# wangxuanx/Face-Diffusion-Model

Measured on AMD Instinct MI355X. Metric: animated frames/sec (1000-step DDPM, VOCASET FDM) at 1/2/4/8 MI355X, higher is better.
Workload: dtype bf16; 1 GPU; cfg2: vocaset FDM, 4 clips/GPU x 200 latent frames, 1000-step DDPM, random-init weights, synthetic audio-encoder features, Philox noise; global_batch=4, latent_frames=200, diffusion_steps=1000, parallelism=clip-shard x1

## Files before the change

### face-diffusion-model_amd/csrc/attention.hpp

```cpp
#pragma once
#include "common.hpp"
#include "../../include/fdm_hip.h"

namespace fdm {

template <typename T> __device__ __forceinline__ float fexp(float x) {
  if constexpr (is_fast16<T>::value) return __builtin_amdgcn_exp2f(x);
  else return expf(x);
}

template <typename T, int HD> constexpr bool attn_streamed() { return Opnd<T>::NP == 2 && HD == 256; }

template <typename T, int HD, int QS, bool RAG = false>
__global__ __launch_bounds__(256, (attn_streamed<T, HD>() ? 1 : 2)) void attn_kernel(const void* pQ, const void* pKp, const void* pVp, int p_q_lo_off, int p_kv_lo_off, int pL, int pB, int pH, int p_ldq,
                                                                                     int pLpad, const fdm_attn_args p) {
  using E = typename Opnd<T>::E;
  constexpr int NP = Opnd<T>::NP;
  constexpr float SCL = Opnd<T>::SCALE;
  constexpr int EPC = 16 / (int)sizeof(E);
  constexpr int NKS = HD / (4 * EPC);
  constexpr int KT = 4 * EPC;
  constexpr int NSUB = KT / 16;
  constexpr int NC = HD / 16;
  constexpr int BQ = 16 * QS;
// ... 162 lines not shown
          pf = __builtin_bit_cast(u32x4, pb);
        } else {
          pf = __builtin_bit_cast(u32x4, sc[0]);
        }
#pragma unroll
        for (int c = 0; c < NC; ++c) Mma<T>::run(o[u][c], vf[c][0], pf);
      } else {
        typedef __attribute__((ext_vector_type(8))) E e8;
        e8 ph, plo;
#pragma unroll
        for (int j = 0; j < 8; ++j) {
          const float x = sc[j >> 2][j & 3];
          const E hi = (E)x;
          ph[j] = hi;
          plo[j] = (E)((x - (float)hi) * SCL);
        }
        const u32x4 pfh = __builtin_bit_cast(u32x4, ph), pfl = __builtin_bit_cast(u32x4, plo);
#pragma unroll
        for (int c = 0; c < NC; ++c) {
          mma16<E>(o[u][c], vf[c][0], pfh);
          mma16<E>(ol[u][c], vf[c][0], pfl);
          mma16<E>(ol[u][c], vf[c][1], pfh);
        }
      }
    }
  }

#pragma unroll
  for (int u = 0; u < QS; ++u) {
    float l_tot = l_part[u];
    l_tot = rows_sum(l_tot);
    if (g == 0) { part_m[wave][16 * u + r16] = m_run[u]; part_l[wave][16 * u + r16] = l_tot; }
#pragma unroll
    for (int c = 0; c < NC; ++c) {
      f32x4 ov = o[u][c];
      if constexpr (NP == 2) ov += ol[u][c] * (1.f / SCL);
      *(f32x4*)&part_o[wave][16 * u + r16][c * 16 + 4 * g] = ov;
    }
  }
  __syncthreads();
  {
    constexpr int TPQ = 256 / BQ;
    constexpr int EPT = HD / TPQ;
    constexpr int RUN = (EPT == 16 && TPQ == 16) ? 8 : EPT;
    const int q = threadIdx.x / TPQ;
    const int e0 = (threadIdx.x % TPQ) * RUN;
    const int qq = q0 + q;
    float mw[4], ms = -INFINITY;
#pragma unroll
    for (int w = 0; w < 4; ++w) { mw[w] = part_m[w][q]; ms = fmaxf(ms, mw[w]); }
    float sw[4], lsum = 0.f;
#pragma unroll
    for (int w = 0; w < 4; ++w) { sw[w] = fexp<T>(mw[w] - ms); lsum += sw[w] * part_l[w][q]; }
    const float inv = 1.f / lsum;
    if (qq < L) {
      const size_t oo = ((size_t)b * L + qq) * p.ldo + (size_t)h * HD + e0;
#pragma unroll
      for (int rr = 0; rr < EPT / RUN; ++rr)
#pragma unroll
      for (int jj = 0; jj < RUN; jj += 4) {
        const int j = rr * TPQ * RUN + jj;
        f32x4 v = f32x4{0.f, 0.f, 0.f, 0.f};
#pragma unroll
        for (int w = 0; w < 4; ++w) v += *(const f32x4*)&part_o[w][q][e0 + j] * sw[w];
        v *= inv;
        if constexpr (RAG) { if (qq >= Lc) v = f32x4{0.f, 0.f, 0.f, 0.f}; }
        if constexpr (std::is_same<T, float>::value) {
          if (p.o_split == FDM_F16X3) store_opnd4<f16x3_t>((f16*)p.O + oo + j, p.o_lo_off, v);
          else *(f32x4*)((float*)p.O + oo + j) = v;
        } else {
          store_opnd4<T>((E*)p.O + oo + j, p.o_lo_off, v);
        }
      }
    }
  }
}

#define ATTN_PRELOAD_ARGS a.Q, a.Kp, a.Vp, (int)a.q_lo_off, (int)a.kv_lo_off, a.L, a.B, a.H, (int)a.ldq, a.Lpad
template <typename T, int HD>
static void attn_launch_t(const fdm_attn_args& a, hipStream_t s) {
  constexpr int qs2 = 384;
  const int groups = (a.B * a.H + 7) / 8 * 8;
  if constexpr (HD <= 128 && Opnd<T>::NP == 1) {
    if (a.L >= qs2) {
      dim3 grid((a.L + 31) / 32 * groups);
      if (a.lens) { hipLaunchKernelGGL((attn_kernel<T, HD, 2, true>), grid, dim3(256), 0, s, ATTN_PRELOAD_ARGS, a); return; }
      hipLaunchKernelGGL((attn_kernel<T, HD, 2>), grid, dim3(256), 0, s, ATTN_PRELOAD_ARGS, a);
      return;
    }
  }
  dim3 grid((a.L + 15) / 16 * groups);
  if constexpr (HD <= 128) {
    if (a.lens) { hipLaunchKernelGGL((attn_kernel<T, HD, 1, true>), grid, dim3(256), 0, s, ATTN_PRELOAD_ARGS, a); return; }
  }
  hipLaunchKernelGGL((attn_kernel<T, HD, 1>), grid, dim3(256), 0, s, ATTN_PRELOAD_ARGS, a);
}

template <typename T>
static hipError_t attn_launch_dtype(const fdm_attn_args& a, hipStream_t s) {
  if (a.lens && a.hd != 64 && a.hd != 128) return hipErrorInvalidValue;
  if constexpr (Opnd<T>::NP == 2) {
    if (a.hd == 256) attn_launch_t<T, 256>(a, s);
    else if (a.hd == 128) attn_launch_t<T, 128>(a, s);
    else if (a.hd == 64) attn_launch_t<T, 64>(a, s);
    else return hipErrorInvalidValue;
  } else {
    if (a.hd == 256) attn_launch_t<T, 256>(a, s);
    else if (a.hd == 128) attn_launch_t<T, 128>(a, s);
    else attn_launch_t<T, 64>(a, s);
  }
  return hipGetLastError();
}

template <typename T>
__global__ void pack_kv_kernel(const T* K, long long ldk, const T* V, long long ldv, T* Kp, T* Vp, int B, int H, int L, int Lpad, int hd) {
  const size_t n = (size_t)B * L * H * hd;
  for (size_t i = (size_t)blockIdx.x * blockDim.x + threadIdx.x; i < n; i += (size_t)gridDim.x * blockDim.x) {
    const int e = (int)(i % hd);
    const int h = (int)((i / hd) % H);
    const size_t row = i / ((size_t)hd * H);
    const int b = (int)(row / L), l = (int)(row % L);
    const size_t blk = (size_t)(b * H + h) * Lpad * hd;
    Kp[blk + kp_offset<T>(l, e, hd)] = K[row * ldk + (size_t)h * hd + e];
    Vp[blk + vp_offset<T>(l, e, hd)] = V[row * ldv + (size_t)h * hd + e];
  }
}
template <typename T>
static hipError_t pack_kv_launch(const void* K, long long ldk, const void* V, long long ldv, void* Kp, void* Vp,
                                 int B, int H, int L, int Lpad, int hd, hipStream_t s) {
  const size_t n = (size_t)B * L * H * hd;
  const int blocks = (int)min((size_t)4096, (n + 255) / 256);
  hipLaunchKernelGGL(pack_kv_kernel<T>, dim3(blocks), dim3(256), 0, s, (const T*)K, ldk, (const T*)V, ldv, (T*)Kp, (T*)Vp, B, H, L, Lpad, hd);
  return hipGetLastError();
}

}
```

### face-diffusion-model_amd/csrc/elementwise.hpp

```cpp
#pragma once
#include "common.hpp"
#include "handoff.hpp"
#include "sched.hpp"
#include "../../include/fdm_hip.h"
#include "host.hpp"

namespace fdm {

template <typename T, int NV, bool HEAVY, bool CLIP = false>
__global__ __launch_bounds__(64 * NV) void ln_row_kernel(const float* p_x, const float* p_add_mat, const float* p_add_tab, const int* p_tab_step,
                                                         const int* p_tab_index, int p_add_mat_group, int p_add_mat_wrap, int p_add_mat_L,
                                                         const fdm_ln_args p) {
  __shared__ float red[4][NV];
  constexpr int d = 256 * NV;
#ifdef FDM_GEMM_STAMPS
  const unsigned long long t_first = wall_clock64();
  unsigned long long t_loaded = 0, t_reduced = 0;
#endif
  const int tid = threadIdx.x, lane = tid & 63, wave = tid >> 6;
  const int row = blockIdx.x, col = tid * 4;
  const bool two = p.gamma2 != nullptr;
  const f32x4 zero = f32x4{0.f, 0.f, 0.f, 0.f};
  f32x4 v = *(const f32x4*)(p_x + (size_t)row * d + col);
  const int npl = p.x_planes;
  f32x4 vpl[3];
#pragma unroll
  for (int i = 0; i < 3; ++i) vpl[i] = (i + 1 < npl) ? *(const f32x4*)(p_x + (size_t)(i + 1) * p.x_plane_stride + (size_t)row * d + col) : zero;
  const bool has_e = p_add_mat || p_add_tab;
  int arow = row;
  if (p_add_mat_group > 0) {
    const int m = p_add_mat_wrap > 0 ? row % p_add_mat_wrap : row;
    arow = (m / p_add_mat_group) * p_add_mat_L + m % p_add_mat_L;
  }
  const f32x4 em = p_add_mat ? *(const f32x4*)(p_add_mat + (size_t)arow * d + col) : zero;
  const f32x4 g1 = *(const f32x4*)(p.gamma + col), b1 = *(const f32x4*)(p.beta + col);
  const float *gp2 = two ? p.gamma2 : p.gamma, *bp2 = two ? p.beta2 : p.beta;
  const f32x4 g2 = *(const f32x4*)(gp2 + col), b2 = *(const f32x4*)(bp2 + col);
  f32x4 et = zero;
  if (p_add_tab) {
    int k;
    if constexpr (CLIP) {
      const int m = p.clip_wrap > 0 ? row % p.clip_wrap : row;
      k = p.clip_step[(size_t)(m / p.clip_rows) * p.clip_step_stride];
    } else {
      k = p_tab_step ? *p_tab_step : 0;
    }
    const int idx = p_tab_index ? p_tab_index[k] : k;
    et = *(const f32x4*)(p_add_tab + (size_t)idx * d + col);
  }
  const f32x4 e = p_add_tab ? em + et : em;
  auto block_sum = [&](float x, int slot) {
    x = wave_sum(x);
    if (lane == 0) red[slot][wave] = x;
    __syncthreads();
    float t = 0.f;
#pragma unroll
    for (int w = 0; w < NV; ++w) t += red[slot][w];
    return t;
  };
#pragma unroll
  for (int i = 0; i < 3; ++i)
    if (i + 1 < npl) v += vpl[i];
  if (!two && has_e) v += e;
#ifdef FDM_GEMM_STAMPS
  asm volatile("" ::"v"(v[0]), "v"(e[0]), "v"(g2[0]), "v"(b2[0]));
  __builtin_amdgcn_sched_barrier(0);
  t_loaded = wall_clock64();
  __builtin_amdgcn_sched_barrier(0);
#endif
  float mean = block_sum((v[0] + v[1]) + (v[2] + v[3]), 0) * (1.f / d);
  v -= mean;
  float var = block_sum((v[0] * v[0] + v[1] * v[1]) + (v[2] * v[2] + v[3] * v[3]), 1) * (1.f / d);
  float rstd = 1.f / sqrtf(var + p.eps);
  if (two) {
    v = v * rstd * g1 + b1;
    if (has_e) v += e;
    mean = block_sum((v[0] + v[1]) + (v[2] + v[3]), 2) * (1.f / d);
    v -= mean;
    var = block_sum((v[0] * v[0] + v[1] * v[1]) + (v[2] * v[2] + v[3] * v[3]), 3) * (1.f / d);
    rstd = 1.f / sqrtf(var + p.eps);
  }
  f32x4 y = v * rstd * g2 + b2;
#ifdef FDM_GEMM_STAMPS
  asm volatile("" ::"v"(y[0]));
  __builtin_amdgcn_sched_barrier(0);
  t_reduced = wall_clock64();
  __builtin_amdgcn_sched_barrier(0);
#endif
  if constexpr (HEAVY) {
#pragma unroll
    for (int j = 0; j < 4; ++j) y[j] = act_apply_t<T>(y[j], p.act);
  } else if (p.act == ACT_RELU) {
#pragma unroll
    for (int j = 0; j < 4; ++j) y[j] = fmaxf(y[j], 0.f);
  }
  if (p.y_f32) st16(p.y_f32 + (size_t)row * d + col, y);
  if (p.y_t) store_opnd4<T>((typename Opnd<T>::E*)p.y_t + (size_t)row * d + col, p.y_t_lo_off, y);
#ifdef FDM_GEMM_STAMPS
  if (p.x_planes == 0 && p.x_plane_stride) {
    const unsigned long long t_issued = wall_clock64();
    asm volatile("s_waitcnt vmcnt(0)" ::: "memory");
    __syncthreads();
    if (tid == 0) {
      unsigned long long* st = (unsigned long long*)p.x_plane_stride + (size_t)row * 8;
      st[5] = t_first; st[0] = t_first; st[1] = t_loaded; st[2] = t_reduced; st[3] = t_issued; st[4] = wall_clock64();
    }
  }
#endif
}

#define LN_PRELOAD_ARGS a.x, a.add_mat, a.add_tab, a.tab_step, a.tab_index, a.add_mat_group, a.add_mat_wrap, a.add_mat_L
template <typename T, bool HEAVY>
static hipError_t ln_launch_h(const fdm_ln_args& a, hipStream_t s) {
  dim3 grid(a.M);
  if constexpr (!HEAVY) {
    if (a.clip_step) {
      switch (a.d) {
        case 256: hipLaunchKernelGGL((ln_row_kernel<T, 1, false, true>), grid, dim3(64), 0, s, LN_PRELOAD_ARGS, a); break;
        case 512: hipLaunchKernelGGL((ln_row_kernel<T, 2, false, true>), grid, dim3(128), 0, s, LN_PRELOAD_ARGS, a); break;
        case 768: hipLaunchKernelGGL((ln_row_kernel<T, 3, false, true>), grid, dim3(192), 0, s, LN_PRELOAD_ARGS, a); break;
        case 1024: hipLaunchKernelGGL((ln_row_kernel<T, 4, false, true>), grid, dim3(256), 0, s, LN_PRELOAD_ARGS, a); break;
        default: return hipErrorInvalidValue;
      }
      return hipGetLastError();
    }
  } else if (a.clip_step) {
    return hipErrorInvalidValue;
  }
  switch (a.d) {
    case 256: hipLaunchKernelGGL((ln_row_kernel<T, 1, HEAVY>), grid, dim3(64), 0, s, LN_PRELOAD_ARGS, a); break;
    case 512: hipLaunchKernelGGL((ln_row_kernel<T, 2, HEAVY>), grid, dim3(128), 0, s, LN_PRELOAD_ARGS, a); break;
    case 768: hipLaunchKernelGGL((ln_row_kernel<T, 3, HEAVY>), grid, dim3(192), 0, s, LN_PRELOAD_ARGS, a); break;
    case 1024: hipLaunchKernelGGL((ln_row_kernel<T, 4, HEAVY>), grid, dim3(256), 0, s, LN_PRELOAD_ARGS, a); break;
    default: return hipErrorInvalidValue;
  }
  return hipGetLastError();
}
template <typename T>
static hipError_t ln_launch_t(const fdm_ln_args& a, hipStream_t s) {
  return (a.act != ACT_NONE && a.act != ACT_RELU) ? ln_launch_h<T, true>(a, s) : ln_launch_h<T, false>(a, s);
}

__global__ __launch_bounds__(256) void sched_kernel(const fdm_sched_args p) {
  const SchedCoef c = p.mode == 3 ? sched_coef_load<true>(p) : sched_coef_load<false>(p);
  const int k = c.k;
  if (p.arrive && p.advance) {
    asm volatile("s_waitcnt vmcnt(0)" ::: "memory");
    __syncthreads();
  }
  if (p.arrive && p.advance && threadIdx.x == 0) {
    const unsigned tk = atomicAdd(p.arrive, 1u);
    if (tk == gridDim.x - 1) {
      *p.arrive = 0u;
      *p.step = k + 1;
    }
  }
  const long long nq = p.n / 4;
  for (long long i = (long long)blockIdx.x * blockDim.x + threadIdx.x; i < nq; i += (long long)gridDim.x * blockDim.x) {
    f32x4 x0 = *(const f32x4*)(p.x0 + 4 * i);
    if (p.x0u) sched_cfg_mix4(x0, *(const f32x4*)(p.x0u + 4 * i), p.cfg_scale);
    f32x4 o;
    if (p.mode == 2) {
      o = x0;
    } else {
      const f32x4 x = *(const f32x4*)(p.x + 4 * i);
      o = sched_update4_rt(p, c, x0, x, 4 * i);
    }
    *(f32x4*)(p.x_out + 4 * i) = o;
    sched_store_t4(p, 4 * i, o);
  }
}

__global__ void step_advance_kernel(int* step) { *step += 1; }

static hipError_t sched_launch(const fdm_sched_args& a, hipStream_t s) {
  hipLaunchKernelGGL(sched_kernel, dim3(grid_for(a.n / 4)), dim3(256), 0, s, a);
  if (a.advance && a.step && !a.arrive) hipLaunchKernelGGL(step_advance_kernel, dim3(1), dim3(1), 0, s, a.step);
  return hipGetLastError();
}

template <typename T>
__global__ void cast_kernel(const float* src, typename Opnd<T>::E* dst, long long n) {
  for (long long i = (long long)blockIdx.x * blockDim.x + threadIdx.x; i < n; i += (long long)gridDim.x * blockDim.x)
    store_opnd1<T>(dst + i, n, src[i]);
}

__global__ void bias_act_kernel(const float* in, const float* vec, float* out, long long rows, int d, int act) {
  const long long n = rows * d;
  for (long long i = (long long)blockIdx.x * blockDim.x + threadIdx.x; i < n; i += (long long)gridDim.x * blockDim.x)
    out[i] = act_apply(in[i] + (vec ? vec[i % d] : 0.f), act);
}

struct AddRowsArgs {
  const float* a; int a_div, a_mod;
  const float* b; int b_div, b_mod;
  const float* c; int c_div, c_mod;
  float* out; long long M; int d;
// ... 620 lines not shown
```

### face-diffusion-model_amd/csrc/fdm_hip.hip

```cpp
#include <hip/hip_runtime.h>

#include <cstdarg>
#include <cstdio>
#include <functional>

#include "elementwise.hpp"
#include "window.hpp"
#include "slots.hpp"
#include "host.hpp"
#include "gemm_tiles.hpp"

namespace fdm {
thread_local std::string g_err;
int fail(int code, const char* fmt, ...) {
  char buf[512];
  va_list ap;
  va_start(ap, fmt);
  vsnprintf(buf, sizeof(buf), fmt, ap);
  va_end(ap);
  g_err = buf;
  return code;
}
}

// ... 71 lines not shown
  if (hipGetDeviceCount(&n) != hipSuccess || n <= 0) return 0;
  hipDeviceProp_t prop;
  if (hipGetDeviceProperties(&prop, 0) != hipSuccess) return 0;
  return strncmp(prop.gcnArchName, "gfx950", 6) == 0 ? 1 : 0;
}

static bool gemm_act_heavy_host(int act) { return act == FDM_ACT_MISH || act == FDM_ACT_GELU_ERF || act == FDM_ACT_GELU_TANH; }

int fdm_op_gemm(const fdm_gemm_args* a, void* stream) {
  if (!a || !a->A || !a->W) return fail(FDM_ERR_ARG, "gemm: null operand");
  if (a->M <= 0 || a->N <= 0 || a->K <= 0) return fail(FDM_ERR_SHAPE, "gemm: M,N,K must be positive (%d,%d,%d)", a->M, a->N, a->K);
  if (!kind_ok(a->dtype)) return fail(FDM_ERR_ARG, "gemm: bad dtype %d", a->dtype);
  const bool split = kind(a->dtype).planes == 2;
  const int bk = kind(a->dtype).bk, epc = kind(a->dtype).epc;
  if (split && (a->a_lo_off <= 0 || a->w_lo_off <= 0 || a->a_lo_off % epc || a->w_lo_off % epc))
    return fail(FDM_ERR_ARG, "gemm: split operands need positive a_lo_off / w_lo_off (multiples of 8 elements)");
  if (split && a->out_t && a->out_t_lo_off <= 0) return fail(FDM_ERR_ARG, "gemm: split out_t needs out_t_lo_off");
  if (a->K % bk) return fail(FDM_ERR_SHAPE, "gemm: K=%d not a multiple of %d", a->K, bk);
  if (a->lda % epc || a->ldw % epc || !aligned16(a->A) || !aligned16(a->W)) return fail(FDM_ERR_ARG, "gemm: operands need 16-byte aligned rows");
  if (a->lda < 0 || a->ldw < 0 || a->lda > 0x7fffffffLL || a->ldw > 0x7fffffffLL) return fail(FDM_ERR_SHAPE, "gemm: lda / ldw are passed to the kernel as 32-bit element counts");
  if (a->a_batch_stride % epc || a->w_batch_stride % epc) return fail(FDM_ERR_ARG, "gemm: batch strides need 16-byte alignment");
  if (!a->out_f32 && !a->out_t && !a->out_vp && !a->out_kp) return fail(FDM_ERR_ARG, "gemm: no output");
  if (a->out_kp || a->out_vp) {
    const int hi = a->out_vp ? a->vp_col0 : a->N;
    if (a->kv_hd <= 0 || a->kv_hd % 16 || a->kv_L <= 0 || a->kv_Lpad < a->kv_L || a->kv_Lpad % 32 || a->M % a->kv_L)
      return fail(FDM_ERR_SHAPE, "gemm: bad packed K/V geometry (hd %d, L %d, Lpad %d)", a->kv_hd, a->kv_L, a->kv_Lpad);
    if (a->out_vp && (a->vp_col0 < 0 || a->vp_col0 % 4 || (a->N - a->vp_col0) % a->kv_hd)) return fail(FDM_ERR_SHAPE, "gemm: bad packed V column range");
    if (a->out_kp && (a->kp_col0 < 0 || a->kp_col0 % 4 || hi < a->kp_col0 || (hi - a->kp_col0) % a->kv_hd)) return fail(FDM_ERR_SHAPE, "gemm: bad packed K column range");
    if (!aligned16(a->out_kp) || !aligned16(a->out_vp)) return fail(FDM_ERR_ARG, "gemm: packed K/V buffers must be 16-byte aligned");
    if (a->dtype == FDM_F16X3 && (a->kv_lo_off <= 0 || a->kv_lo_off % 8)) return fail(FDM_ERR_ARG, "gemm: split packed K/V outputs need kv_lo_off");
  }
  if (a->bias && !aligned16(a->bias)) return fail(FDM_ERR_ARG, "gemm: bias must be 16-byte aligned");
  if (a->ln_stat_in && (a->ln_nparts <= 0 || a->ln_dim <= 0)) return fail(FDM_ERR_ARG, "gemm: ln_stat_in needs ln_nparts and ln_dim");
  if ((a->ln_colsum || a->rln_gamma) && !a->ln_stat_in) return fail(FDM_ERR_ARG, "gemm: LayerNorm folding needs ln_stat_in");
  if (a->rln_gamma && (!a->rln_beta || !a->resid)) return fail(FDM_ERR_ARG, "gemm: rln_gamma needs rln_beta and resid");
  if ((a->stat_out || a->ln_stat_in) && (a->batch > 1 || a->out_batch_stride)) return fail(FDM_ERR_ARG, "gemm: LayerNorm folding is not batched");
  if (a->tile < 0 || (a->tile & FDM_TILE_ID_MASK) > FDM_TILE_MAX) return fail(FDM_ERR_ARG, "gemm: unknown tile %d", a->tile);
  if (a->sched_fuse) {
    const fdm_sched_args& sc = a->sched;
    if (sc.mode != 0 && sc.mode != 1 && sc.mode != 3) return fail(FDM_ERR_ARG, "gemm: fused scheduler supports mode 0 (DDPM), 1 (DDIM) and 3 (table-driven)");
    if (!a->resid || !a->out_f32 || a->N % 64 || a->ldo_f32 != a->N || a->ldr != a->N || a->resid_row_mod || a->batch > 1 ||
        !aligned16(a->resid) || !aligned16(a->out_f32) || (a->out_t && (a->ldo_t != a->N || !aligned16(a->out_t))))
      return fail(FDM_ERR_SHAPE, "gemm: fused scheduler needs resid = x_t and out_f32 = x_{t-1} as dense [M, N] arrays, N %% 64 == 0");
    if (gemm_act_heavy_host(a->act) || a->stat_out || a->out_kp || a->out_vp || a->rln_gamma)
      return fail(FDM_ERR_ARG, "gemm: fused scheduler cannot be combined with Mish/GELU, stat_out, packed K/V or rln outputs");
    if (sc.mode == 0 && (!sc.c1 || !sc.c2 || !sc.sigma)) return fail(FDM_ERR_ARG, "gemm: fused DDPM needs c1, c2, sigma");
    if (sc.mode == 1 && (!sc.sra || !sc.srm1 || !sc.sqrt_an || !sc.c_n)) return fail(FDM_ERR_ARG, "gemm: fused DDIM needs sra, srm1, sqrt_an, c_n");
    if (sc.mode == 0 && !sc.noise && sc.n_per_clip <= 0) return fail(FDM_ERR_ARG, "gemm: fused DDPM with Philox noise needs n_per_clip");
    if (sc.mode == 3 && (!sc.lm_a || !sc.lm_b || !sc.lm_c || !sc.lm_s || !sc.x0_hist || !aligned16(sc.x0_hist)))
      return fail(FDM_ERR_ARG, "gemm: fused table-driven sampler needs lm_a, lm_b, lm_c, lm_s and a 16-byte aligned x0_hist [M, N]");
    if (sc.mode == 3 && !sc.noise && sc.n_per_clip <= 0) return fail(FDM_ERR_ARG, "gemm: fused table-driven sampler with Philox noise needs n_per_clip");
  }
  if (a->ksplit < 0 || a->ksplit > 4) return fail(FDM_ERR_ARG, "gemm: ksplit %d outside 0..4", a->ksplit);
  if (a->ksplit > 1) {
    const int tl = a->tile & FDM_TILE_ID_MASK;
    if (a->batch > 1 || a->out_batch_stride || a->act != FDM_ACT_NONE || !a->out_f32 || a->out_t || a->out_kp || a->out_vp || a->stat_out || a->ln_stat_in ||
        a->sched_fuse || a->resid_row_mod || (a->tile & FDM_TILE_GENERAL))
      return fail(FDM_ERR_ARG, "gemm: ksplit needs a plain launch (one batch, no activation, out_f32 as the only output, no folds)");
    if ((a->K / bk) % a->ksplit) return fail(FDM_ERR_SHAPE, "gemm: ksplit %d does not divide the %d k-tiles of K=%d", a->ksplit, a->K / bk, a->K);
    if (a->N % 64 || a->ldo_f32 % 4 || !aligned16(a->out_f32) || a->ksplit_stride % 4 || a->ksplit_stride < (long long)(a->M - 1) * a->ldo_f32 + a->N ||
        (a->resid && (a->ldr % 4 || !aligned16(a->resid))))
      return fail(FDM_ERR_SHAPE, "gemm: ksplit needs N %% 64 == 0, 16-byte aligned rows and ksplit_stride >= one output plane");
    if (tl != 0 && !gemm_tile_can(tl, TILE_KSPLIT))
      return fail(FDM_ERR_ARG, "gemm: ksplit runs on the 64-column tiles (FDM_TILE_64x64, FDM_TILE_64x64_S2, FDM_TILE_32x64_S3), not tile %d", tl);
  }
  if (a->batch2 < 0) return fail(FDM_ERR_ARG, "gemm: negative batch2");
  if (a->batch2 >= 1) {
    const int tl = a->tile & FDM_TILE_ID_MASK;
    if (a->ksplit > 1 || a->out_kp || a->out_vp || a->stat_out || a->ln_stat_in || a->sched_fuse || a->resid_row_mod || a->incr_counter)
      return fail(FDM_ERR_ARG, "gemm: batch2 cannot be combined with ksplit, packed K/V, LayerNorm folds, the fused scheduler or resid_row_mod");
    if (a->a_batch_stride2 % epc) return fail(FDM_ERR_ARG, "gemm: a_batch_stride2 needs 16-byte alignment");
    if (tl != 0 && !gemm_tile_can(tl, TILE_BATCH2))
      return fail(FDM_ERR_ARG, "gemm: batch2 runs on the 64-column tiles (FDM_TILE_64x64, FDM_TILE_64x64_S2, FDM_TILE_128x64), not tile %d", tl);
    if (a->batch < 1) return fail(FDM_ERR_ARG, "gemm: batch2 needs batch >= 1 (the group count of the second batch level)");
  }
  fdm_gemm_args c = *a;
  return submit([c](hipStream_t s) { return fdm::gemm_launch(c, s); }, stream, "gemm");
}

int fdm_gemm_heuristic_tile(const fdm_gemm_args* a) {
  if (!a) return fail(FDM_ERR_ARG, "gemm_heuristic_tile: null argument");
  fdm_gemm_args b = *a;
  b.tile = 0;
  if (b.batch2 >= 1 && b.ksplit <= 1 && !b.sched_fuse && gemm_tile_override() > 0) return gemm_tile_override();
  return gemm_requested_tile(b);
}

int fdm_op_attention(const fdm_attn_args* a, void* stream) {
  if (!a || !a->Q || !a->Kp || !a->Vp || !a->O) return fail(FDM_ERR_ARG, "attention: null operand");
  if (a->hd != 64 && a->hd != 128 && a->hd != 256) return fail(FDM_ERR_SHAPE, "attention: head_dim %d unsupported (64, 128, 256)", a->hd);
  if (a->B <= 0 || a->H <= 0 || a->L <= 0) return fail(FDM_ERR_SHAPE, "attention: B,H,L must be positive");
  if (a->Lpad < a->L || a->Lpad % 32) return fail(FDM_ERR_SHAPE, "attention: Lpad=%d must be a multiple of 32 >= L", a->Lpad);
  if (!kind_ok(a->dtype)) return fail(FDM_ERR_ARG, "attention: bad dtype %d (FDM_F32, FDM_BF16, FDM_F16X3, FDM_F16)", a->dtype);
  if (a->o_split && (a->dtype != FDM_F32 || a->o_split != FDM_F16X3 || a->o_lo_off <= 0))
    return fail(FDM_ERR_ARG, "attention: o_split needs dtype FDM_F32, a split kind and o_lo_off");
  if (a->dtype == FDM_F16X3 && (a->q_lo_off <= 0 || a->kv_lo_off <= 0 || a->o_lo_off <= 0 || a->q_lo_off % 8 || a->kv_lo_off % 8 || a->o_lo_off % 4))
    return fail(FDM_ERR_ARG, "attention: split operands need q_lo_off, kv_lo_off and o_lo_off");
  if (a->q_lo_off > 0x7fffffffLL || a->kv_lo_off > 0x7fffffffLL || a->ldq > 0x7fffffffLL)
    return fail(FDM_ERR_SHAPE, "attention: q_lo_off, kv_lo_off and ldq are passed to the kernel as 32-bit element counts");
  const int epc = kind(a->dtype).epc;
  if (a->ldq % epc || a->ldo % 4 || !aligned16(a->Q) || !aligned16(a->Kp) || !aligned16(a->Vp) || !aligned16(a->O))
    return fail(FDM_ERR_ARG, "attention: operands need 16-byte aligned rows");
  if (a->slopes && a->period <= 0) return fail(FDM_ERR_ARG, "attention: period must be positive");
  if (a->lens && (a->causal || (a->hd != 64 && a->hd != 128)))
    return fail(FDM_ERR_ARG, "attention: per-clip lengths need causal = 0 and head_dim 64 or 128");
  fdm_attn_args c = *a;
  return submit([c](hipStream_t s) { return fdm::attn_launch(c, s); }, stream, "attention");
}

int fdm_op_pack_kv(const void* K, long long ldk, const void* V, long long ldv, void* Kp, void* Vp,
                   int B, int H, int L, int Lpad, int hd, int dtype, void* stream) {
  if (!K || !V || !Kp || !Vp) return fail(FDM_ERR_ARG, "pack_kv: null operand");
  if (B <= 0 || H <= 0 || L <= 0 || Lpad < L || Lpad % 32 || hd <= 0 || hd % 16) return fail(FDM_ERR_SHAPE, "pack_kv: bad geometry");
  if (dtype != FDM_F32 && dtype != FDM_BF16) return fail(FDM_ERR_ARG, "pack_kv: bad dtype %d", dtype);
  return submit([=](hipStream_t s) {
    return dtype == FDM_BF16 ? fdm::pack_kv_launch_bf16(K, ldk, V, ldv, Kp, Vp, B, H, L, Lpad, hd, s)
                             : fdm::pack_kv_launch_f32(K, ldk, V, ldv, Kp, Vp, B, H, L, Lpad, hd, s);
  }, stream, "pack_kv");
}

int fdm_op_layernorm(const fdm_ln_args* a, void* stream) {
  if (!a || !a->x || !a->gamma || !a->beta) return fail(FDM_ERR_ARG, "layernorm: null operand");
  if (a->d != 256 && a->d != 512 && a->d != 768 && a->d != 1024) return fail(FDM_ERR_SHAPE, "layernorm: d=%d unsupported (256, 512, 768, 1024)", a->d);
  if (a->M <= 0) return fail(FDM_ERR_SHAPE, "layernorm: M must be positive");
  if (!a->y_f32 && !a->y_t) return fail(FDM_ERR_ARG, "layernorm: no output");
  if (!kind_ok(a->dtype)) return fail(FDM_ERR_ARG, "layernorm: bad dtype %d", a->dtype);
  if (a->y_t && a->dtype == FDM_F16X3 && (a->y_t_lo_off <= 0 || a->y_t_lo_off % 4)) return fail(FDM_ERR_ARG, "layernorm: split y_t needs y_t_lo_off");
  if (a->add_mat_group < 0 || a->add_mat_wrap < 0 ||
      (a->add_mat_group > 0 && (a->add_mat_L <= 0 || a->add_mat_group % a->add_mat_L || (a->add_mat_wrap > 0 && a->add_mat_wrap % a->add_mat_group))))
    return fail(FDM_ERR_SHAPE, "layernorm: shared add_mat needs add_mat_L | add_mat_group | add_mat_wrap (got %d, %d, %d)", a->add_mat_L, a->add_mat_group, a->add_mat_wrap);
  if (a->x_planes < 0 || a->x_planes > 4 || (a->x_planes > 1 && (a->x_plane_stride < (long long)a->M * a->d || a->x_plane_stride % 4)))
    return fail(FDM_ERR_ARG, "layernorm: x_planes %d (0..4) needs x_plane_stride >= M * d, a multiple of 4", a->x_planes);
  if (a->clip_step && (a->clip_rows <= 0 || a->clip_step_stride <= 0 || a->clip_wrap < 0 || (a->clip_wrap > 0 && a->clip_wrap % a->clip_rows)))
    return fail(FDM_ERR_SHAPE, "layernorm: clip_step needs clip_rows > 0, clip_step_stride > 0 and clip_rows | clip_wrap (got %d, %d, %d)", a->clip_rows, a->clip_step_stride, a->clip_wrap);
  if (a->clip_step && a->act != FDM_ACT_NONE && a->act != FDM_ACT_RELU) return fail(FDM_ERR_ARG, "layernorm: clip_step runs with FDM_ACT_NONE / FDM_ACT_RELU only");
  fdm_ln_args c = *a;
  return submit([c](hipStream_t s) {
    switch (c.dtype) {
      case FDM_BF16: return fdm::ln_launch_t<fdm::bf16>(c, s);
      case FDM_F16X3: return fdm::ln_launch_t<fdm::f16x3_t>(c, s);
      case FDM_F16: return fdm::ln_launch_t<fdm::f16>(c, s);
      default: return fdm::ln_launch_t<float>(c, s);
    }
  }, stream, "layernorm");
}

int fdm_op_sched_step(const fdm_sched_args* a, void* stream) {
  if (!a || !a->x0 || !a->x_out) return fail(FDM_ERR_ARG, "sched: null operand");
  if (a->n <= 0 || a->n % 4) return fail(FDM_ERR_SHAPE, "sched: n=%lld must be a positive multiple of 4", a->n);
  if (a->mode == 0 && (!a->x || !a->c1 || !a->c2 || !a->sigma)) return fail(FDM_ERR_ARG, "sched: DDPM tables missing");
  if (a->mode == 1 && (!a->x || !a->sra || !a->srm1 || !a->sqrt_an || !a->c_n)) return fail(FDM_ERR_ARG, "sched: DDIM tables missing");
  if (a->mode == 3 && (!a->x || !a->lm_a || !a->lm_b || !a->lm_c || !a->lm_s || !a->x0_hist)) return fail(FDM_ERR_ARG, "sched: table-driven sampler needs lm_a, lm_b, lm_c, lm_s, x0_hist");
  if (a->mode < 0 || a->mode > 3) return fail(FDM_ERR_ARG, "sched: bad mode %d", a->mode);
  if (a->mode == 3 && !a->noise && (a->n_per_clip <= 0 || a->n_per_clip % 4)) return fail(FDM_ERR_SHAPE, "sched: n_per_clip must be a positive multiple of 4");
  if (a->mode == 0 && !a->noise && (a->n_per_clip <= 0 || a->n_per_clip % 4)) return fail(FDM_ERR_SHAPE, "sched: n_per_clip must be a positive multiple of 4");
  if (a->x_out_t && !kind_ok(a->out_dtype)) return fail(FDM_ERR_ARG, "sched: bad out_dtype %d", a->out_dtype);
  if (a->x_out_t && a->out_dtype == FDM_F16X3 && (a->x_out_t_lo_off <= 0 || a->x_out_t_lo_off % 4)) return fail(FDM_ERR_ARG, "sched: split x_out_t needs x_out_t_lo_off");
  fdm_sched_args c = *a;
  return submit([c](hipStream_t s) { return fdm::sched_launch(c, s); }, stream, "sched");
}

static int check_bank(const fdm_slot_bank_args* b, const char* who) {
  if (!b || !b->req || !b->desc || !b->t) return fail(FDM_ERR_ARG, "%s: null bank table", who);
  if (b->n_samplers < 1 || b->n_t < 1 || b->n_coef < 0 || (b->n_coef > 0 && !b->coef)) return fail(FDM_ERR_SHAPE, "%s: bank sizes (%d samplers, %d timesteps, %d coefficients)", who, b->n_samplers, b->n_t, b->n_coef);
  if (!aligned16(b->req) || !aligned16(b->desc)) return fail(FDM_ERR_ARG, "%s: request rows and descriptors must be 16-byte aligned", who);
  return FDM_OK;
}

static int check_slot_pass(const fdm_sched_args* a, const int* state, const unsigned long long* keys, int n_slots, const fdm_slot_group_args* g,
                           const fdm_slot_bank_args* b, const char* who) {
  if (!a || !a->x_out || !state || !keys || (!g && (!a->x0 || !a->x))) return fail(FDM_ERR_ARG, "%s: null operand", who);
  if (b) FCK(check_bank(b, who));
  if (g) {
    if (!g->member || !g->frames || !g->entries || !g->groups || !g->x_long) return fail(FDM_ERR_ARG, "%s: null table or arena", who);
    if (!g->init && (!a->x0 || !a->x)) return fail(FDM_ERR_ARG, "%s: null operand", who);
    if (g->init && g->plain) return fail(FDM_ERR_ARG, "%s: init loads the arena into the window rows only (plain must be 0)", who);
  }
  const bool own_sampler = !b && !(g && g->init);
  if (a->noise) return fail(FDM_ERR_ARG, "%s: injected noise is not supported (Philox keyed per slot%s)", who, g ? " / group" : "");
  if (own_sampler && a->mode != 0 && a->mode != 1 && a->mode != 3) return fail(FDM_ERR_ARG, "%s: mode %d (0 DDPM, 1 DDIM, 3 table-driven)", who, a->mode);
  if (n_slots < 1 || a->n_per_clip <= 0 || a->n_per_clip % 4 || a->n != (long long)n_slots * a->n_per_clip)
    return fail(FDM_ERR_SHAPE, "%s: n=%lld must be n_slots=%d x n_per_clip=%lld (a multiple of 4)", who, a->n, n_slots, a->n_per_clip);
  if (g) {
    if (g->L < 1 || g->d < 4 || g->d % 4 || (long long)g->L * g->d != a->n_per_clip)
      return fail(FDM_ERR_SHAPE, "%s: L=%d x d=%d (a multiple of 4) must be n_per_clip=%lld", who, g->L, g->d, a->n_per_clip);
    if (g->arena_frames < 1 || g->n_groups < 1 || g->n_entries < 1 || g->frame0 < 0 || g->frame1 < g->frame0 || g->frame1 > g->arena_frames)
      return fail(FDM_ERR_SHAPE, "%s: arena frames [%d, %d) outside [0, %d), or no groups / entries", who, g->frame0, g->frame1, g->arena_frames);
  }
  if (own_sampler) {
    if (a->mode == 0 && (!a->c1 || !a->c2 || !a->sigma)) return fail(FDM_ERR_ARG, "%s: DDPM tables missing", who);
    if (a->mode == 1 && (!a->sra || !a->srm1 || !a->sqrt_an || !a->c_n)) return fail(FDM_ERR_ARG, "%s: DDIM tables missing", who);
    if (a->mode == 3 && (!a->lm_a || !a->lm_b || !a->lm_c || !a->lm_s || !a->x0_hist || (g && !g->hist_long)))
      return fail(FDM_ERR_ARG, "%s: table-driven sampler needs lm_a, lm_b, lm_c, lm_s, x0_hist%s", who, g ? " and hist_long" : "");
  }
  if (a->x_out_t && !kind_ok(a->out_dtype)) return fail(FDM_ERR_ARG, "%s: bad out_dtype %d", who, a->out_dtype);
  if (a->x_out_t && a->out_dtype == FDM_F16X3 && (a->x_out_t_lo_off <= 0 || a->x_out_t_lo_off % 4)) return fail(FDM_ERR_ARG, "%s: split x_out_t needs x_out_t_lo_off", who);
  if (!aligned16(a->x0) || !aligned16(a->x0u) || !aligned16(a->x) || !aligned16(a->x_out) || !aligned16(a->x_out_t) || !aligned16(a->x0_hist) || !aligned16(state) ||
      (g && (!aligned16(g->frames) || !aligned16(g->entries) || !aligned16(g->groups) || !aligned16(g->x_long) || !aligned16(g->hist_long))))
    return fail(FDM_ERR_ARG, "%s: operands%s and the state words must be 16-byte aligned", who, g ? ", table rows" : "");
  return FDM_OK;
}
static const fdm_slot_bank_args no_bank = {};

static fdm_sched_args slot_pass_args(const fdm_sched_args* a, bool bank) {
  fdm_sched_args c = *a;
  c.noise = nullptr; c.step = nullptr; c.tseq = nullptr; c.seed_dev = nullptr; c.arrive = nullptr;
  if (bank) { c.sqrt_an = c.c_n = nullptr; c.lm_a = c.lm_b = c.lm_c = c.lm_s = nullptr; }
  return c;
}

int fdm_op_slot_sched(const fdm_sched_args* a, const int* state, const unsigned long long* keys, int n_slots, void* stream) {
  FCK(check_slot_pass(a, state, keys, n_slots, nullptr, nullptr, "slot_sched"));
  const fdm_sched_args c = slot_pass_args(a, false);
  return submit([c, state, keys](hipStream_t s) { return fdm::slot_sched_launch(c, state, keys, nullptr, s); }, stream, "slot_sched");
}

int fdm_op_slot_group_sched(const fdm_sched_args* a, const int* state, const unsigned long long* keys, int n_slots,
                            const fdm_slot_group_args* g, void* stream) {
// ... 495 lines not shown
```

### face-diffusion-model_amd/csrc/plan.hip

```cpp
#include <hip/hip_runtime.h>

#include <cmath>
#include <cstdio>

#include "common.hpp"
#include "plan.hpp"

std::string fdm::shape_key(const fdm_plan* P) {
  char b[80];
  snprintf(b, sizeof(b), "%d,%d,%d,%d,%d,ks%d.%d", P->R, P->M, P->L, P->rep, P->S, P->ksplit_out, P->ksplit_ffn2);
  return b;
}

int fdm::drop_programs(fdm_plan* P, void* stream) {
  if (P->progs.empty()) return FDM_OK;
  if (stream) HIPCK(hipStreamSynchronize((hipStream_t)stream));
  else HIPCK(hipDeviceSynchronize());
  for (auto& kv : P->progs) fdm_prog_destroy(kv.second);
  P->progs.clear();
  P->prog_order.clear();
  P->pinned.clear();
  return FDM_OK;
}

namespace {
using namespace fdm;

__global__ void transpose_kernel(const float* in, float* out, int rows, int cols) {
  const long long n = (long long)rows * cols;
  for (long long i = (long long)blockIdx.x * blockDim.x + threadIdx.x; i < n; i += (long long)gridDim.x * blockDim.x) {
    const int c = (int)(i / rows), r = (int)(i % rows);
    out[i] = in[(size_t)r * cols + c];
  }
}
__global__ void scale_cols_kernel(const float* W, const float* gamma, float* out, long long n, int K) {
  for (long long i = (long long)blockIdx.x * blockDim.x + threadIdx.x; i < n; i += (long long)gridDim.x * blockDim.x)
    out[i] = W[i] * gamma[i % K];
}
__global__ __launch_bounds__(256) void rowsum_bf16_kernel(const fdm::bf16* W, float* out, int N, int K) {
  const int lane = threadIdx.x & 63, row = blockIdx.x * 4 + (threadIdx.x >> 6);
  if (row >= N) return;
  float s = 0.f;
  for (int k = lane; k < K; k += 64) s += (float)W[(size_t)row * K + k];
  s = fdm::wave_sum(s);
  if (lane == 0) out[row] = s;
}
template <typename E>
__global__ __launch_bounds__(256) void rowsum_split_kernel(const E* W, long long lo_off, float inv_scale, float* out, int N, int K) {
  const int lane = threadIdx.x & 63, row = blockIdx.x * 4 + (threadIdx.x >> 6);
  if (row >= N) return;
  float s = 0.f;
  for (int k = lane; k < K; k += 64) s += (float)W[(size_t)row * K + k] + (float)W[lo_off + (size_t)row * K + k] * inv_scale;
  s = fdm::wave_sum(s);
  if (lane == 0) out[row] = s;
}

template <typename T> int zalloc(Arena& a, T** out, size_t n) { return a.alloc_t(out, n, true); }
int zalloc_mat(const fdm_plan* P, Arena& a, Mat* out, size_t rows, size_t cols) {
  const size_t n = rows * cols;
  out->lo = kind(P->dtype).planes == 2 ? (long long)n : 0;
  return a.alloc(&out->p, n * kind(P->dtype).full(), true);
}

const Wt* weight(const fdm_plan* P, const std::string& name) {
  auto it = P->w.find(name);
  return it == P->w.end() ? nullptr : &it->second;
}
int need(const fdm_plan* P, const std::string& name, long long n, const float** out) { return need_weight(P->w, "plan: ", name, n, out); }

fdm_gemm_args gemm_op(const fdm_plan* P, const Mat& A, const Mat& W, int M, int N, int K) {
  fdm_gemm_args a = dense_gemm(P->dtype, A.p, W.p, M, N, K);
  a.a_lo_off = A.lo; a.w_lo_off = W.lo;
  return a;
}
void set_out_t(fdm_gemm_args& a, const Mat& o) { a.out_t = o.p; a.out_t_lo_off = o.lo; }

void set_ln_stats(fdm_gemm_args& g, const fdm_plan* P) { g.ln_stat_in = P->stats; g.ln_nparts = P->m.d / 64; g.ln_dim = P->m.d; g.ln_eps = 1e-5f; }
void set_ksplit(fdm_gemm_args& g, int S, long long plane) { if (S > 1) { g.ksplit = S; g.ksplit_stride = plane; } }
void set_ksplit(fdm_ln_args& ln, int S, long long plane) { if (S > 1) { ln.x_planes = S; ln.x_plane_stride = plane; } }

int plan_gemm(fdm_plan* P, const char* label, fdm_gemm_args a, void* stream) {
  if (P->tune_rec) (*P->tune_rec)[label].push_back(a);
  auto it = P->tiles.find(label);
  a.tile = (it == P->tiles.end() ? 0 : it->second) | (P->lockstep ? FDM_TILE_LOCKSTEP : 0);
  return fdm_op_gemm(&a, stream);
}

std::string lname(int l, const char* suffix) {
  char b[96];
  snprintf(b, sizeof(b), "transformer_decoder.layers.%d.%s", l, suffix);
  return b;
}

int commit_impl(fdm_plan* P, void* stream) {
  const fdm_model_desc& m = P->m;
  const int d = m.d;
  hipStream_t s = (hipStream_t)stream;
  FCK(drop_programs(P, stream));
  const float* p = nullptr;
  FCK(need(P, "audio_extract.0.weight", (long long)d * m.audio_in, &p));
  FCK(need(P, "audio_extract.0.bias", d, &p));
  FCK(need(P, "audio_extract.2.weight", (long long)d * d, &p));
  FCK(need(P, "audio_extract.2.bias", d, &p));
  FCK(need(P, "style_embedd.weight", (long long)d * m.n_style, &p));
  FCK(need(P, "style_embedd.bias", d, &p));
  if (m.n_emo) { FCK(need(P, "emotion_embedd.weight", (long long)d * m.n_emo, &p)); FCK(need(P, "emotion_embedd.bias", d, &p)); }
  FCK(need(P, "latent_encoder.0.bias", d, &p));
  FCK(need(P, "latent_decoder.bias", d, &p));
  std::vector<std::pair<std::string, long long>> mats = {{"latent_encoder.0.weight", (long long)d * d}, {"latent_decoder.weight", (long long)d * d}};
  for (int l = 0; l < m.n_layers; ++l) {
    mats.push_back({lname(l, "self_attn.in_proj_weight"), 3LL * d * d});
    mats.push_back({lname(l, "self_attn.out_proj.weight"), (long long)d * d});
    mats.push_back({lname(l, "linear1.weight"), (long long)m.ffn * d});
    mats.push_back({lname(l, "linear2.weight"), (long long)d * m.ffn});
    for (const char* b : {"self_attn.in_proj_bias", "self_attn.out_proj.bias", "linear1.bias", "linear2.bias", "norm1.weight", "norm1.bias",
                          "norm2.weight", "norm2.bias", "norm3.weight", "norm3.bias"}) {
      const long long nb = !strcmp(b, "self_attn.in_proj_bias") ? 3LL * d : (!strcmp(b, "linear1.bias") ? m.ffn : d);
      FCK(need(P, lname(l, b), nb, &p));
    }
  }
  for (auto& mt : mats) {
    FCK(need(P, mt.first, mt.second, &p));
    Mat o;
    FCK(to_operand(P->cmem, P->dtype, p, mt.second, &o, stream));
    P->wt[mt.first] = o;
  }
  const float *Wt_ = nullptr, *bt = nullptr;
  FCK(need(P, "time_embedd.0.weight", (long long)d * 1000, &Wt_));
  FCK(need(P, "time_embedd.0.bias", d, &bt));
  float* wtT = nullptr;
  FCK(zalloc(P->cmem, &wtT, (size_t)1000 * d));
  FCK(zalloc(P->cmem, &P->tau, (size_t)1000 * d));
  hipLaunchKernelGGL(transpose_kernel, dim3(grid_for(1000LL * d)), dim3(256), 0, s, Wt_, wtT, d, 1000);
  FCK(fdm_op_bias_act(wtT, bt, P->tau, 1000, d, FDM_ACT_MISH, stream));
  float* tmp = nullptr;
  FCK(zalloc(P->cmem, &tmp, (size_t)1000 * d));
  P->TT.assign(m.n_layers, nullptr);
  P->Wv.assign(m.n_layers, nullptr); P->bv = P->Wo = P->bo = P->Wv;
  for (int l = 0; l < m.n_layers; ++l) {
    const float *ipw = nullptr, *ipb = nullptr;
    FCK(need(P, lname(l, "multihead_attn.in_proj_weight"), 3LL * d * d, &ipw));
    FCK(need(P, lname(l, "multihead_attn.in_proj_bias"), 3LL * d, &ipb));
    FCK(need(P, lname(l, "multihead_attn.out_proj.weight"), (long long)d * d, &P->Wo[l]));
    FCK(need(P, lname(l, "multihead_attn.out_proj.bias"), d, &P->bo[l]));
    P->Wv[l] = ipw + 2LL * d * d;
    P->bv[l] = ipb + 2LL * d;
    FCK(zalloc(P->cmem, &P->TT[l], (size_t)1000 * d));
    fdm_gemm_args g = dense_gemm(FDM_F32, P->tau, P->Wv[l], 1000, d, d);
    g.out_f32 = tmp;
    FCK(fdm_op_gemm(&g, stream));
    g = dense_gemm(FDM_F32, tmp, P->Wo[l], 1000, d, d);
    g.out_f32 = P->TT[l];
    FCK(fdm_op_gemm(&g, stream));
  }
  P->fuse_ln3 = (P->dtype == FDM_BF16 || P->dtype == FDM_F16X3) && P->want_fuse_ln3;
  if (P->fuse_ln3) {
    auto make_fold = [&](const std::string& wname, const std::string& bname, int N, int l_prev, Fold* f) -> int {
      const float *W = nullptr, *b = nullptr, *gam = nullptr, *bet = nullptr;
      FCK(need(P, wname, (long long)N * d, &W));
      FCK(need(P, bname, N, &b));
      FCK(need(P, lname(l_prev, "norm3.weight"), d, &gam));
      FCK(need(P, lname(l_prev, "norm3.bias"), d, &bet));
// ... 80 lines not shown
  FCK(drop_programs(P, nullptr));
  P->ws.release();
  P->prepared = false;
  const fdm_model_desc& m = P->m;
  const size_t d = m.d, M = (size_t)B * L, R = M * repc;
  const size_t Lpad = ((size_t)L + 31) / 32 * 32;
  FCK(zalloc(P->ws, &P->h, R * d)); FCK(zalloc(P->ws, &P->h2, R * d)); P->x1_planes = std::max(1, std::max(P->ksplit_out, P->ksplit_ffn2));
  FCK(zalloc(P->ws, &P->x1, R * d * P->x1_planes));
  FCK(zalloc(P->ws, &P->x0, R * d)); FCK(zalloc(P->ws, &P->x, M * d));
  FCK(zalloc(P->ws, &P->x0_hist, M * d));
  if (P->dtype != FDM_F32) {
    FCK(zalloc_mat(P, P->ws, &P->xt, M, d)); FCK(zalloc_mat(P, P->ws, &P->ht, R, d)); FCK(zalloc_mat(P, P->ws, &P->h2t, R, d));
  } else {
    P->xt = Mat{P->x, 0}; P->ht = Mat{P->h, 0}; P->h2t = Mat{P->h2, 0};
  }
  if (P->dtype != FDM_F32) {
    FCK(zalloc(P->ws, &P->x2, R * d)); FCK(zalloc_mat(P, P->ws, &P->x2t, R, d)); FCK(zalloc(P->ws, &P->stats, (d / 64) * R * 2));
  }
  const size_t ea = kind(P->dtype).full();
  FCK(P->ws.alloc(&P->q, R * d * ea, true));
  FCK(P->ws.alloc(&P->kp, (size_t)B * repc * Lpad * d * ea, true));
  FCK(P->ws.alloc(&P->vp, (size_t)B * repc * Lpad * d * ea, true));
  P->q_lo = (long long)(R * d);
  P->kv_lo = (long long)((size_t)B * repc * Lpad * d);
  P->kv_bytes = (size_t)B * repc * Lpad * d * ea;
  FCK(zalloc_mat(P, P->ws, &P->ctx, R, d));
  FCK(zalloc_mat(P, P->ws, &P->u, R, m.ffn));
  FCK(zalloc(P->ws, &P->AF, M * d)); FCK(zalloc(P->ws, &P->t1, M * d));
  FCK(zalloc(P->ws, &P->sty, (size_t)B * d)); FCK(zalloc(P->ws, &P->em, (size_t)B * d)); FCK(zalloc(P->ws, &P->emu, (size_t)B * d));
  FCK(zalloc(P->ws, &P->zeros, (size_t)B * (m.n_emo > 0 ? m.n_emo : 1)));
  FCK(zalloc(P->ws, &P->E0, R * d));
  P->C1.assign(m.n_layers, nullptr);
  for (int l = 0; l < m.n_layers; ++l) FCK(zalloc(P->ws, &P->C1[l], R * d));
  FCK(zalloc(P->ws, &P->step, (size_t)4));
  FCK(zalloc(P->ws, &P->seedbuf, (size_t)2));
  if (!P->tseq) { P->tseq_cap = 1024; FCK(zalloc(P->mem, &P->tseq, (size_t)P->tseq_cap)); }
  if (!P->lm_tab) { P->lm_cap = 1024; FCK(zalloc(P->mem, &P->lm_tab, (size_t)4 * P->lm_cap)); }
  P->capB = B; P->capL = L; P->capRep = repc;
  return FDM_OK;
}

}

int fdm::record_chain(fdm_plan* P, const fdm_sched_args* sched, void* stream) {
  const fdm_model_desc& m = P->m;
  const int d = m.d, M = P->M, R = P->R, L = P->L;
  const bool both = P->dtype != FDM_F32, split = kind(P->dtype).planes == 2, fuse = P->fuse_ln3;
  int* step = P->step; int* tcur = P->step + 1;
  const float *b = nullptr;
  {
    FCK(need(P, "latent_encoder.0.bias", d, &b));
    fdm_gemm_args g = gemm_op(P, P->xt, P->wt["latent_encoder.0.weight"], M, d, d);
    g.bias = b; g.act = m.latent_mish ? FDM_ACT_MISH : FDM_ACT_NONE;
    g.resid = P->E0; g.out_f32 = P->h;
    if (both) set_out_t(g, P->ht);
    g.batch = P->rep; g.out_batch_stride = (long long)M * d;
    if (!P->slots) { g.incr_counter = step; g.incr_table = P->tseq; }
    FCK(plan_gemm(P, "enc", g, stream));
  }
  const int BB = P->B * P->rep;
  const float eps = 1e-5f;
  for (int l = 0; l < m.n_layers; ++l) {
    const Fold* f = (fuse && l > 0) ? &P->fold[l] : nullptr;
    fdm_gemm_args g;
    if (!f) {
      FCK(need(P, lname(l, "self_attn.in_proj_bias"), 3LL * d, &b));
      g = gemm_op(P, P->ht, P->wt[lname(l, "self_attn.in_proj_weight")], R, 3 * d, d);
      g.bias = b;
    } else {
      g = gemm_op(P, P->x2t, f->w, R, 3 * d, d);
      g.bias = f->bias; g.ln_colsum = f->colsum; set_ln_stats(g, P);
    }
    g.out_t = P->q; g.ldo_t = d; g.out_t_lo_off = split ? P->q_lo : 0;
    g.kv_lo_off = split ? P->kv_lo : 0;
    g.out_kp = P->kp; g.kp_col0 = d; g.out_vp = P->vp; g.vp_col0 = 2 * d; g.kv_L = L; g.kv_Lpad = P->Lpad; g.kv_hd = P->hd;
    FCK(plan_gemm(P, f ? "qkv_ln" : "qkv", g, stream));
    fdm_attn_args at;
    memset(&at, 0, sizeof(at));
    at.Q = P->q; at.ldq = d;
    at.Kp = P->kp; at.Vp = P->vp; at.Lpad = P->Lpad; at.O = P->ctx.p; at.ldo = d;
    at.B = BB; at.H = m.n_head; at.L = L; at.hd = P->hd; at.dtype = P->dtype;
    at.scale = 1.0f / std::sqrt((float)P->hd); at.causal = 1; at.slopes = P->slopes; at.period = m.period;
    if (split) { at.q_lo_off = P->q_lo; at.kv_lo_off = P->kv_lo; at.o_lo_off = P->ctx.lo; }
    FCK(fdm_op_attention(&at, stream));
    FCK(need(P, lname(l, "self_attn.out_proj.bias"), d, &b));
    g = gemm_op(P, P->ctx, P->wt[lname(l, "self_attn.out_proj.weight")], R, d, d);
    g.bias = b; g.out_f32 = P->x1;
    if (!f) {
      g.resid = P->h;
      set_ksplit(g, P->ksplit_out, (long long)R * d);
      FCK(plan_gemm(P, "out", g, stream));
    } else {
      g.resid = P->x2; g.rln_gamma = f->gamma; g.rln_beta = f->beta; set_ln_stats(g, P);
      FCK(plan_gemm(P, "out_ln", g, stream));
    }
    fdm_ln_args ln;
    memset(&ln, 0, sizeof(ln));
    ln.x = P->x1; ln.M = R; ln.d = d; ln.add_mat = P->C1[l]; ln.add_tab = P->TT[l]; ln.tab_step = tcur; ln.eps = eps;
    if (P->S > 1) { ln.add_mat_L = L; ln.add_mat_group = P->S * L; ln.add_mat_wrap = M; }
    if (P->slots) {
      ln.tab_step = nullptr; ln.clip_step = P->slot_state + 1; ln.clip_step_stride = 4; ln.clip_rows = L; ln.clip_wrap = M;
    }
    if (!f) set_ksplit(ln, P->ksplit_out, (long long)R * d);
    FCK(need(P, lname(l, "norm1.weight"), d, &ln.gamma)); FCK(need(P, lname(l, "norm1.bias"), d, &ln.beta));
    FCK(need(P, lname(l, "norm2.weight"), d, &ln.gamma2)); FCK(need(P, lname(l, "norm2.bias"), d, &ln.beta2));
    ln.y_f32 = P->h2; ln.dtype = P->dtype;
    if (both) { ln.y_t = P->h2t.p; ln.y_t_lo_off = P->h2t.lo; }
    FCK(fdm_op_layernorm(&ln, stream));
    FCK(need(P, lname(l, "linear1.bias"), m.ffn, &b));
    g = gemm_op(P, P->h2t, P->wt[lname(l, "linear1.weight")], R, m.ffn, d);
    g.bias = b; g.act = FDM_ACT_RELU; set_out_t(g, P->u);
    FCK(plan_gemm(P, "ffn1", g, stream));
    FCK(need(P, lname(l, "linear2.bias"), d, &b));
    g = gemm_op(P, P->u, P->wt[lname(l, "linear2.weight")], R, d, m.ffn);
    g.bias = b; g.resid = P->h2;
    if (fuse) {
      g.out_f32 = P->x2; set_out_t(g, P->x2t); g.stat_out = P->stats;
      FCK(plan_gemm(P, "ffn2_stat", g, stream));
    } else {
      g.out_f32 = P->x1;
      set_ksplit(g, P->ksplit_ffn2, (long long)R * d);
      FCK(plan_gemm(P, "ffn2", g, stream));
      memset(&ln, 0, sizeof(ln));
      ln.x = P->x1; ln.M = R; ln.d = d; ln.eps = eps; ln.y_f32 = P->h; ln.dtype = P->dtype;
      set_ksplit(ln, P->ksplit_ffn2, (long long)R * d);
      FCK(need(P, lname(l, "norm3.weight"), d, &ln.gamma)); FCK(need(P, lname(l, "norm3.bias"), d, &ln.beta));
      if (both) { ln.y_t = P->ht.p; ln.y_t_lo_off = P->ht.lo; }
      FCK(fdm_op_layernorm(&ln, stream));
    }
  }
  fdm_gemm_args g;
  if (fuse) {
    const Fold& f = P->fold[-1];
    g = gemm_op(P, P->x2t, f.w, R, d, d);
    g.bias = f.bias; g.ln_colsum = f.colsum; set_ln_stats(g, P);
  } else {
    FCK(need(P, "latent_decoder.bias", d, &b));
    g = gemm_op(P, P->ht, P->wt["latent_decoder.weight"], R, d, d);
    g.bias = b;
  }
  if (sched) {
    g.resid = P->x; g.out_f32 = P->x;
    if (both) set_out_t(g, P->xt);
    g.sched_fuse = 1; g.sched = *sched;
  } else {
    g.out_f32 = P->x0;
  }
  return plan_gemm(P, fuse ? "dec_ln" : "dec", g, stream);
}

namespace {

struct ProgSpec {
  int kind;
  const float* noise = nullptr; float cfg_scale = 0.f;
  const float* san = nullptr; const float* cn = nullptr;
  int reps = 1;
  int slot_steps = 0;
  int bank = 0;
};

std::string tiles_sig(const fdm_plan* P) {
  std::string s;
  for (auto& kv : P->tiles)
    if (kv.second) s += kv.first + "=" + std::to_string(kv.second) + ",";
  s += "ks" + std::to_string(P->ksplit_out) + std::to_string(P->ksplit_ffn2) + (P->lockstep ? "L" : "");
  return s;
}

fdm::WinArgs win_args(const fdm_plan* P, int init) {
  fdm::WinArgs w;
  w.off = P->win_off; w.ent = P->win_ent; w.xw = P->x;
  w.L_total = P->win_total; w.n_win = P->win_n; w.W = P->win_len; w.d = P->m.d; w.init = init;
  return w;
}

fdm_slot_group_args long_args(const fdm_plan* P, int f0, int f1, int plain, int init) {
  fdm_slot_group_args g;
  memset(&g, 0, sizeof(g));
  g.member = P->slot_member; g.frames = (const int*)P->long_frame; g.entries = P->long_ent; g.groups = (const int*)P->long_group;
  g.x_long = P->long_x; g.hist_long = P->long_hist;
  g.arena_frames = P->long_frames; g.n_entries = P->long_entries; g.n_groups = P->long_groups;
  g.L = P->L; g.d = P->m.d; g.frame0 = f0; g.frame1 = f1; g.plain = plain; g.init = init;
  return g;
}

fdm_slot_bank_args bank_args(const fdm_plan* P) {
  fdm_slot_bank_args b;
  memset(&b, 0, sizeof(b));
  b.req = P->slot_req; b.desc = P->bank_desc; b.t = P->bank_t; b.coef = P->bank_c;
  b.n_samplers = P->bank_rows; b.n_t = P->bank_t_cap; b.n_coef = P->bank_c_cap;
  return b;
}

int get_program(fdm_plan* P, const ProgSpec& sp, void* stream, fdm_prog** out) {
  char key[512];
  snprintf(key, sizeof(key), "%s#%s|%d|%p|%a|%p|%d", shape_key(P).c_str(), tiles_sig(P).c_str(), sp.kind, (const void*)sp.noise, (double)sp.cfg_scale,
           (const void*)sp.san, sp.reps);
  if (P->win_n) {
    const size_t kl = strlen(key);
    snprintf(key + kl, sizeof(key) - kl, "|win%d,%d,%d,%d,%d", P->win_B, P->win_total, P->win_n, P->win_len, P->win_overlap);
  }
  if (P->slots) {
    const size_t kl = strlen(key);
    snprintf(key + kl, sizeof(key) - kl, "|slot%d,%d,%p", sp.slot_steps, P->slots, (const void*)sp.cn);
    if (P->long_frames) {
      const size_t k2 = strlen(key);
      snprintf(key + k2, sizeof(key) - k2, "|long%d,%d", P->long_frames, P->long_groups);
    }
    if (sp.bank) {
      const size_t k3 = strlen(key);
      snprintf(key + k3, sizeof(key) - k3, "|bank%d,%d,%d", P->bank_rows, P->bank_t_cap, P->bank_c_cap);
    }
  }
  auto it = P->progs.find(key);
  if (it != P->progs.end()) {
    auto pos = std::find(P->prog_order.begin(), P->prog_order.end(), std::string(key));
    if (pos != P->prog_order.end()) { P->prog_order.erase(pos); P->prog_order.push_back(key); }
    P->pinned.push_back(key);
    if (sp.reps == 1) P->launches_per_step = fdm_prog_num_ops(it->second);
    *out = it->second;
    return FDM_OK;
  }
  if (P->progs.size() >= 16) {
    auto victim = P->prog_order.end();
    for (auto v = P->prog_order.begin(); v != P->prog_order.end(); ++v)
      if (std::find(P->pinned.begin(), P->pinned.end(), *v) == P->pinned.end()) { victim = v; break; }
    if (victim != P->prog_order.end()) {
      HIPCK(hipStreamSynchronize((hipStream_t)stream));
      const std::string vk = *victim;
      P->prog_order.erase(victim);
      fdm_prog_destroy(P->progs[vk]);
      P->progs.erase(vk);
    }
  }
  const int d = P->m.d, M = P->M;
  const long long n = (long long)M * d;
  fdm_prog* prog = nullptr;
  FCK(fdm_prog_create(&prog));
  int rc = fdm_prog_begin(prog);
  const bool fuse_sched = !P->cfg && sp.kind != 0 && !sp.slot_steps;
  for (int rep = 0; rc == FDM_OK && rep < sp.reps; ++rep) {
    fdm_sched_args sc;
    memset(&sc, 0, sizeof(sc));
    sc.x0 = P->x0; sc.x0u = P->cfg ? P->x0 + n : nullptr; sc.cfg_scale = sp.cfg_scale;
    sc.x = P->x; sc.x_out = P->x; sc.n = n; sc.tseq = P->tseq; sc.step = P->step; sc.advance = 0;
    if (P->dtype != FDM_F32) { sc.x_out_t = P->xt.p; sc.out_dtype = P->dtype; sc.x_out_t_lo_off = P->xt.lo; }
    if (sp.kind == 1) {
// ... 931 lines not shown
  }
  g = fdm_plan::GroupHost();
  return FDM_OK;
}

int fdm_slot_sampler_add(fdm_plan* P, const fdm_sample_args* a, void* stream) {
  if (!a) return fail(FDM_ERR_ARG, "slot_sampler_add: null sampler");
  if (a->noise || a->record) return fail(FDM_ERR_ARG, "slot_sampler_add: injected noise and record are not supported in slot mode");
  if (!P) return fail(FDM_ERR_ARG, "slot_sampler_add: null plan");
  FCK(check_slots(P, "slot_sampler_add"));
  SamplerDef def;
  FCK(sampler_def(a, "slot_sampler_add", def));
  if (def.ts.empty()) return fail(FDM_ERR_ARG, "slot_sampler_add: the sampler has no live step (ddim_steps = %d)", a->ddim_steps);
  if (!P->bank_rows) return fail(FDM_ERR_STATE, "slot_sampler_add: the session has no sampler bank (fdm_plan_set slot_samplers / slot_sampler_steps before fdm_slots_open)");
  int id = -1;
  for (int i = 1; i < P->bank_rows && id < 0; ++i)
    if (!P->sampler_host[i].used) id = i;
  if (id < 0) return fail(FDM_ERR_STATE, "slot_sampler_add: all %d bank rows are in use", P->bank_rows - 1);
  auto first_fit = [&](bool coef, int need, int cap) {
    std::vector<std::pair<int, int>> used;
    for (const auto& h : P->sampler_host)
      if (h.used && (coef ? h.n_c : h.n_steps) > 0) used.push_back(coef ? std::make_pair(h.c_off, h.n_c) : std::make_pair(h.t_off, h.n_steps));
    std::sort(used.begin(), used.end());
    int at = 0;
    for (const auto& u : used) {
      if (u.first - at >= need) return at;
      at = u.first + u.second;
    }
    return cap - at >= need ? at : -1;
  };
  const int nt = (int)def.ts.size(), nc = (int)def.coef.size();
  const int t_off = first_fit(false, nt, P->bank_t_cap), c_off = nc ? first_fit(true, nc, P->bank_c_cap) : 0;
  if (t_off < 0) return fail(FDM_ERR_STATE, "slot_sampler_add: no free range of %d timesteps (bank %d)", nt, P->bank_t_cap);
  if (c_off < 0) return fail(FDM_ERR_STATE, "slot_sampler_add: no free range of %d coefficients (bank %d)", nc, P->bank_c_cap);
  hipStream_t s = (hipStream_t)stream;
  const int desc[4] = {def.mode, nt, t_off, c_off};
  HIPCK(hipMemcpyAsync(P->bank_t + t_off, def.ts.data(), (size_t)nt * 4, hipMemcpyHostToDevice, s));
  if (nc) HIPCK(hipMemcpyAsync(P->bank_c + c_off, def.coef.data(), (size_t)nc * 4, hipMemcpyHostToDevice, s));
  HIPCK(hipMemcpyAsync(P->bank_desc + 4 * (size_t)id, desc, 16, hipMemcpyHostToDevice, s));
  HIPCK(hipStreamSynchronize(s));
  fdm_plan::SamplerHost& h = P->sampler_host[id];
  h.used = true; h.kind = def.kind; h.mode = def.mode; h.n_steps = nt; h.t0 = def.ts[0]; h.t_off = t_off; h.c_off = c_off; h.n_c = nc;
  return id;
}

int fdm_slot_sampler_drop(fdm_plan* P, int id) {
  if (!P) return fail(FDM_ERR_ARG, "slot_sampler_drop: null plan");
  FCK(check_slots(P, "slot_sampler_drop"));
  if (id < 1 || id >= P->bank_rows || !P->sampler_host[id].used) return fail(FDM_ERR_ARG, "slot_sampler_drop: %s", id == 0 ? "sampler 0 belongs to the session" : "unknown sampler");
  for (size_t i = 0; i < P->slot_host.size(); ++i)
    if (P->slot_host[i].status != 0 && P->slot_host[i].sampler == id)
      return fail(FDM_ERR_STATE, "slot_sampler_drop: slot %d (%s) names sampler %d", (int)i, P->slot_host[i].status == 1 ? "running" : "finished and not read", id);
  P->sampler_host[id] = fdm_plan::SamplerHost();
  return FDM_OK;
}

int fdm_slot_sampler_info(fdm_plan* P, int id, int* kind, int* n_steps) {
  if (!P) return fail(FDM_ERR_ARG, "slot_sampler_info: null plan");
  FCK(check_slots(P, "slot_sampler_info"));
  if (!P->bank_rows) {
    if (id != 0) return fail(FDM_ERR_ARG, "slot_sampler_info: unknown sampler %d", id);
    if (kind) *kind = P->slot_kind - 1;
    if (n_steps) *n_steps = P->slot_nsteps;
    return FDM_OK;
  }
  if (id < 0 || id >= P->bank_rows || !P->sampler_host[id].used) return fail(FDM_ERR_ARG, "slot_sampler_info: unknown sampler %d", id);
  if (kind) *kind = P->sampler_host[id].kind;
  if (n_steps) *n_steps = P->sampler_host[id].n_steps;
  return FDM_OK;
}

int fdm_plan_tune(fdm_plan* P, void* stream) {
  FCK(check_ready(P));
  return tune_tiles(P, 1, stream);
}

int fdm_plan_get(fdm_plan* P, const char* key, long long* out) {
  if (!P || !key || !out) return fail(FDM_ERR_ARG, "plan_get: null argument");
  const std::string k(key);
  if (k == "launches_per_step") *out = P->launches_per_step;
  else if (k == "graph_launches") *out = P->last_graph_launches;
  else if (k == "fuse_ln3") *out = P->fuse_ln3;
  else if (k == "rows") *out = P->R;
  else if (k == "ksplit.out") *out = P->ksplit_out;
  else if (k == "ksplit.ffn2") *out = P->ksplit_ffn2;
  else if (k == "tuned") *out = P->tile_cache.count(shape_key(P)) ? 1 : 0;
  else if (k == "needs_tune") *out = needs_tune(P, shape_key(P)) ? 1 : 0;
  else if (k == "tune_failed") *out = P->tune_failed;
  else if (k == "windows") *out = P->win_n;
  else if (k == "slots") *out = P->slots;
  else if (k == "slot_long_frames") *out = P->want_long_frames;
  else if (k == "slot_long_groups") *out = P->want_long_groups;
  else if (k == "slot_samplers") *out = P->want_samplers;
  else if (k == "slot_sampler_steps") *out = P->want_sampler_steps;
  else if (k == "window_len") *out = P->win_n ? P->win_len : P->L;
  else if (k == "L_total") *out = P->win_n ? P->win_total : P->L;
  else if (k.rfind("tile.", 0) == 0) { auto it = P->tiles.find(k.substr(5)); *out = it == P->tiles.end() ? 0 : it->second; }
  else return fail(FDM_ERR_ARG, "plan_get: unknown key '%s'", key);
  return FDM_OK;
}

int fdm_plan_set(fdm_plan* P, const char* key, long long value) {
  if (!P || !key) return fail(FDM_ERR_ARG, "plan_set: null argument");
  const std::string k(key);
  if (k == "tune") { P->tune_enabled = value != 0; return FDM_OK; }
  if (k == "tune_lazy") { P->tune_lazy = value != 0; return FDM_OK; }
  if (k == "slot_long_frames" || k == "slot_long_groups") {
    if (value < 0 || value > 0x3fffffffLL) return fail(FDM_ERR_ARG, "plan_set: %s = %lld", key, value);
    (k == "slot_long_frames" ? P->want_long_frames : P->want_long_groups) = (int)value;
    return FDM_OK;
  }
  if (k == "slot_samplers" || k == "slot_sampler_steps") {
    if (value < 0 || value > 0xfffffLL) return fail(FDM_ERR_ARG, "plan_set: %s = %lld", key, value);
    (k == "slot_samplers" ? P->want_samplers : P->want_sampler_steps) = (int)value;
    return FDM_OK;
  }
  if (k == "fuse_ln3") {
    if ((value != 0) != (P->want_fuse_ln3 != 0)) { P->want_fuse_ln3 = value != 0; P->committed = false; P->prepared = false; return drop_programs(P, nullptr); }
    return FDM_OK;
  }
  if (k == "ksplit.out" || k == "ksplit.ffn2") {
    const int kt = (k == "ksplit.out" ? P->m.d : P->m.ffn) / kind(P->dtype).bk;
    if (value < 1 || value > 4 || kt % value) return fail(FDM_ERR_ARG, "plan_set: %s = %lld must be 1..4 and divide the %d k-tiles", key, value, kt);
    int& cur = k == "ksplit.out" ? P->ksplit_out : P->ksplit_ffn2;
    if (cur == (int)value) return FDM_OK;
    cur = (int)value;
    P->tile_cache.clear(); P->tiles.erase(k == "ksplit.out" ? "out" : "ffn2");
    FCK(drop_programs(P, nullptr));
    if (P->capB > 0 && (int)value > P->x1_planes) {
      P->x1_planes = (int)value;
      FCK(zalloc(P->ws, &P->x1, (size_t)P->capB * P->capL * P->capRep * P->m.d * P->x1_planes));
    }
    return FDM_OK;
  }
  if (k == "lockstep") { P->lockstep = value != 0; P->tile_cache.clear(); P->tiles.clear(); return drop_programs(P, nullptr); }
  if (k == "untune") {
    P->tile_cache.clear(); P->steps_seen.clear(); P->tiles.clear(); P->tune_failed_shapes.clear();
    return drop_programs(P, nullptr);
  }
  if (k.rfind("tile.", 0) == 0) {
    if (value < 0 || value > FDM_TILE_MAX) return fail(FDM_ERR_ARG, "plan_set: unknown tile %lld", value);
    P->tiles[k.substr(5)] = (int)value;
    P->tile_cache[shape_key(P)] = P->tiles;
    return drop_programs(P, nullptr);
  }
  return fail(FDM_ERR_ARG, "plan_set: unknown key '%s'", key);
}

}
```

### face-diffusion-model_amd/csrc/plan.hpp

```cpp
#pragma once
#include <set>

#include "host.hpp"

struct Fold { fdm::Mat w; float* colsum = nullptr; float* bias = nullptr; const float* gamma = nullptr; const float* beta = nullptr; };

struct fdm_plan {
  fdm_model_desc m{};
  int dtype = FDM_F32, hd = 0;
  fdm::Arena mem, ws, cmem;
  std::map<std::string, fdm::Wt> w;
  bool committed = false;
  std::map<std::string, fdm::Mat> wt;
  float* tau = nullptr;
  std::vector<float*> TT;
  std::vector<const float*> Wv, bv, Wo, bo;
  bool fuse_ln3 = false;
  std::map<int, Fold> fold;
  float *slopes = nullptr, *pe = nullptr;
  float *c1 = nullptr, *c2 = nullptr, *sigma = nullptr, *sra = nullptr, *srm1 = nullptr;
  int capB = 0, capL = 0, capRep = 0;
  int B = 0, L = 0, M = 0, rep = 1, R = 0, Lpad = 0, cfg = 0;
  int S = 1;
  bool prepared = false;
  float *h = nullptr, *h2 = nullptr, *x1 = nullptr, *x0 = nullptr, *x = nullptr, *x2 = nullptr, *stats = nullptr;
  fdm::Mat xt, ht, h2t, x2t, ctx, u;
  void *q = nullptr, *kp = nullptr, *vp = nullptr;
  long long q_lo = 0, kv_lo = 0;
  size_t kv_bytes = 0;
  float *AF = nullptr, *t1 = nullptr, *sty = nullptr, *em = nullptr, *emu = nullptr, *zeros = nullptr, *E0 = nullptr;
  std::vector<float*> C1;
  int* step = nullptr;
  unsigned long long* seedbuf = nullptr;
  int* tseq = nullptr; int tseq_cap = 0;
  float* lm_tab = nullptr; int lm_cap = 0;
  float* x0_hist = nullptr;
  std::map<int, std::pair<int, float*>> ddim;
  std::map<int, std::vector<int>> ddim_t;
  std::map<std::string, fdm_prog*> progs;
  std::vector<std::string> prog_order;
  std::vector<std::string> pinned;
  std::map<std::string, int> tiles;
  std::map<std::string, std::map<std::string, int>> tile_cache;
  std::map<std::string, long long> steps_seen;
  std::map<std::string, std::vector<fdm_gemm_args>>* tune_rec = nullptr;
  int tune_enabled = 1;
  int tune_failed = 0;
  std::set<std::string> tune_failed_shapes;
  int want_fuse_ln3 = 0;
  int ksplit_out = 1, ksplit_ffn2 = 1;
  int x1_planes = 0;
  int lockstep = 0;
  int tune_lazy = 0;
  long long last_graph_launches = 0, launches_per_step = 0;
  int win_n = 0, win_len = 0, win_total = 0, win_overlap = 0, win_B = 0;
  float* xlong = nullptr; size_t xlong_cap = 0;
  float* hist_long = nullptr; size_t hist_long_cap = 0;
  int* win_off = nullptr; size_t win_off_cap = 0;
  fdm::WinEnt* win_ent = nullptr; size_t win_ent_cap = 0;
  float* win_stage = nullptr; size_t win_stage_cap = 0;
  int slots = 0;
  int* slot_state = nullptr; size_t slot_state_cap = 0;
  unsigned long long* slot_keys = nullptr; size_t slot_keys_cap = 0;
  struct SlotHost { int status = 0, done = 0, L = 0, group = -1, sampler = 0, total = 0; };
  std::vector<SlotHost> slot_host;
  int slot_kind = 0, slot_nsteps = 0, slot_t0 = 0;
  int slot_graph_steps = 0, slot_eager = 0;
  float slot_cfg_scale = 0.f;
  const float *slot_san = nullptr, *slot_cn = nullptr;
  int want_long_frames = 0, want_long_groups = 0;
  int long_frames = 0, long_groups = 0, long_entries = 0;
  float* long_x = nullptr; size_t long_x_cap = 0;
  float* long_hist = nullptr; size_t long_hist_cap = 0;
  fdm::LongFrame* long_frame = nullptr; size_t long_frame_cap = 0;
  fdm::LongEnt* long_ent = nullptr; size_t long_ent_cap = 0;
  fdm::LongGroup* long_group = nullptr; size_t long_group_cap = 0;
  int* slot_member = nullptr; size_t slot_member_cap = 0;
  struct GroupHost { bool used = false; int L_total = 0, first = 0, e0 = 0, ne = 0; std::vector<int> slots; };
  std::vector<GroupHost> group_host;
  int want_samplers = 0, want_sampler_steps = 0;
  int bank_rows = 0, bank_t_cap = 0, bank_c_cap = 0;
  void* slot_req = nullptr; size_t slot_req_cap = 0;
  int* bank_desc = nullptr; size_t bank_desc_cap = 0;
  int* bank_t = nullptr; size_t bank_t_bytes = 0;
  float* bank_c = nullptr; size_t bank_c_bytes = 0;
  struct SamplerHost { bool used = false; int kind = 0, mode = 0, n_steps = 0, t0 = 0, t_off = 0, c_off = 0, n_c = 0; };
  std::vector<SamplerHost> sampler_host;
};

namespace fdm {
std::string shape_key(const fdm_plan* P);
int drop_programs(fdm_plan* P, void* stream);
int record_chain(fdm_plan* P, const fdm_sched_args* sched, void* stream);
bool needs_tune(fdm_plan* P, const std::string& key);
int tune_tiles(fdm_plan* P, int force, void* stream);
void tune_soft(fdm_plan* P, void* stream);
void select_tiles(fdm_plan* P);
}
```

### face-diffusion-model_amd/csrc/tune.hip

```cpp
#include <cstdio>
#include <cstdlib>
#include <fstream>

#include <unistd.h>

#include "gemm_tiles.hpp"
#include "plan.hpp"

namespace {
using namespace fdm;

int time_prog(fdm_prog* prog, int warm, int reps, hipStream_t s, float* ms) {
  hipEvent_t e0, e1;
  HIPCK(hipEventCreate(&e0)); HIPCK(hipEventCreate(&e1));
  int rc = fdm_prog_instantiate(prog, s);
  if (rc == FDM_OK) rc = fdm_prog_replay(prog, warm, s);
  if (rc == FDM_OK) {
    (void)hipEventRecord(e0, s);
    rc = fdm_prog_replay(prog, reps, s);
    (void)hipEventRecord(e1, s);
    (void)hipEventSynchronize(e1);
    (void)hipEventElapsedTime(ms, e0, e1);
  }
  (void)hipEventDestroy(e0); (void)hipEventDestroy(e1);
  return rc;
}

std::vector<std::pair<std::string, int>> parse_tiles(const std::string& v) {
  std::vector<std::pair<std::string, int>> out;
  size_t pos = 0;
  while (pos < v.size()) {
    const size_t comma = v.find(',', pos), eq = v.find('=', pos);
    const size_t end = comma == std::string::npos ? v.size() : comma;
    if (eq != std::string::npos && eq < end) out.push_back({v.substr(pos, eq - pos), atoi(v.substr(eq + 1, end - eq - 1).c_str())});
    pos = end + 1;
  }
  return out;
}

void apply_tile_override(std::map<std::string, int>& tiles) {
  if (const char* ov = getenv("FDM_TILE_OVERRIDE"))
    for (auto& kv : parse_tiles(ov)) tiles[kv.first] = kv.second;
}

std::string store_key(const fdm_plan* P) {
  const fdm_model_desc& m = P->m;
  char b[160];
  snprintf(b, sizeof(b), "v%d|dt%d|%d,%d,%d,%d,%d,%d,%d,%d|%s", fdm_version(), P->dtype, m.d, m.n_head, m.n_layers, m.ffn, m.G, m.c, m.audio_in, m.pair,
           shape_key(P).c_str());
  return b;
}

bool store_read(std::map<std::string, std::string>& lines) {
  const char* path = getenv("FDM_TILE_CACHE");
  if (!path || !*path) return false;
  std::ifstream f(path);
  std::string ln;
  while (f && std::getline(f, ln)) {
    const size_t tab = ln.find('\t');
    if (tab != std::string::npos) lines[ln.substr(0, tab)] = ln.substr(tab + 1);
  }
  return true;
}

bool store_lookup(const fdm_plan* P, std::map<std::string, int>& tiles) {
  std::map<std::string, std::string> lines;
  if (!store_read(lines)) return false;
  auto it = lines.find(store_key(P));
  if (it == lines.end()) return false;
  tiles.clear();
  for (auto& kv : parse_tiles(it->second)) {
    if (kv.second < 0 || kv.second > FDM_TILE_MAX) return false;
    if (kv.second) tiles[kv.first] = kv.second;
  }
  return true;
}

void store_save(const fdm_plan* P, const std::map<std::string, int>& tiles) {
  std::map<std::string, std::string> lines;
  if (!store_read(lines)) return;
  std::string v;
  for (auto& kv : tiles)
    if (kv.second) v += (v.empty() ? "" : ",") + kv.first + "=" + std::to_string(kv.second);
  lines[store_key(P)] = v;
  const std::string path = getenv("FDM_TILE_CACHE"), tmp = path + ".tmp" + std::to_string((long long)getpid());
  {
    std::ofstream f(tmp, std::ios::trunc);
    if (!f) return;
    for (auto& kv : lines) f << kv.first << '\t' << kv.second << '\n';
  }
  if (rename(tmp.c_str(), path.c_str()) != 0) remove(tmp.c_str());
}

bool tuning_on(const fdm_plan* P) {
  const char* env = getenv("FDM_TUNE");
  return P->tune_enabled && !(env && !strcmp(env, "0"));
}

int tune_tiles_impl(fdm_plan* P, void* stream) {
  const std::string key = shape_key(P);
  hipStream_t s = (hipStream_t)stream;
  const Kind& kd = kind(P->dtype);
  const bool split = kd.planes == 2;
  FCK(drop_programs(P, stream));
  P->tiles.clear();
  std::map<std::string, std::vector<fdm_gemm_args>> calls;
  {
    fdm_prog* dry = nullptr;
    FCK(fdm_prog_create(&dry));
    int rc = fdm_prog_begin(dry);
    P->tune_rec = &calls;
    if (rc == FDM_OK) rc = record_chain(P, nullptr, stream);
    P->tune_rec = nullptr;
    (void)fdm_prog_end(dry);
    fdm_prog_destroy(dry);
    FCK(rc);
  }
  auto timed = [&](const std::vector<fdm_gemm_args>& inst, int tile, float* best) -> int {
    *best = 1e30f;
    for (int rep = 0; rep < 3; ++rep) {
      fdm_prog* prog = nullptr;
      FCK(fdm_prog_create(&prog));
      int rc = fdm_prog_begin(prog);
      for (size_t i = 0; rc == FDM_OK && i < inst.size(); ++i) { fdm_gemm_args a = inst[i]; a.tile = tile | (P->lockstep ? FDM_TILE_LOCKSTEP : 0); a.incr_counter = nullptr; a.incr_table = nullptr; rc = fdm_op_gemm(&a, stream); }
      (void)fdm_prog_end(prog);
      float ms = 0.f;
      if (rc == FDM_OK) rc = time_prog(prog, 2, 5, s, &ms);
      HIPCK(hipStreamSynchronize(s));
      fdm_prog_destroy(prog);
      FCK(rc);
      if (ms < *best) *best = ms;
    }
    return FDM_OK;
  };
  std::vector<int> cands;
  for (const GemmTile& t : kGemmTiles)
    if (gemm_tile_runs(t.id, split) == t.id && !(t.pp && P->R < 1024)) cands.push_back(t.id);
  auto modelled_us = [&](const fdm_gemm_args& a, int tile) {
    const GemmTile& g = gemm_tile(tile);
    const double planes = kd.planes, eb = kd.bytes;
    const long long tiles = (long long)((a.M + g.bm - 1) / g.bm) * ((a.N + g.bn - 1) / g.bn) * (a.batch > 0 ? a.batch : 1);
    const long long rounds = (tiles + 255) / 256;
    const double bytes = (double)rounds * (g.bm + g.bn) * a.K * eb * planes;
    return 5.0 + bytes / 70e3;
  };
  std::map<std::string, int> tuned, runner_up;
  for (auto& kv : calls) {
    std::vector<fdm_gemm_args> inst = kv.second;
    while (inst.size() < 4) { auto c = inst; inst.insert(inst.end(), c.begin(), c.end()); }
    float base = 0.f;
    FCK(timed(inst, 0, &base));
    std::vector<std::pair<float, int>> cand = {{base * 0.97f, 0}};
    double best_model = 1e30;
    for (int tile : cands) best_model = std::min(best_model, modelled_us(kv.second[0], tile));
    auto launched = [&](int tile) { fdm_gemm_args a = kv.second[0]; a.tile = tile; return gemm_resolve_tile(a); };
    const int heur = launched(0);
    const unsigned form = (kv.second[0].ksplit > 1 ? TILE_KSPLIT : 0) | (kv.second[0].sched_fuse ? TILE_SCHED : 0);
    for (int tile : cands) {
      if (launched(tile) == heur) continue;
      if (!gemm_tile_can(tile, form)) continue;
      if (modelled_us(kv.second[0], tile) > 1.35 * best_model) continue;
      float t = 0.f;
      FCK(timed(inst, tile, &t));
      cand.push_back({t, tile});
    }
    std::sort(cand.begin(), cand.end());
    tuned[kv.first] = cand[0].second;
    if (cand.size() > 1 && cand[1].first < cand[0].first * 1.05f) runner_up[kv.first] = cand[1].second;
  }
  auto chain_time = [&](const std::map<std::string, int>& tiles, float* best) -> int {
    *best = 1e30f;
    for (int rep = 0; rep < 2; ++rep) {
      P->tiles = tiles;
      const int init[2] = {-1, 0};
      HIPCK(hipMemcpyAsync(P->step, init, 8, hipMemcpyHostToDevice, s));
      fdm_prog* prog = nullptr;
      FCK(fdm_prog_create(&prog));
      int rc = fdm_prog_begin(prog);
      if (rc == FDM_OK) rc = record_chain(P, nullptr, stream);
      (void)fdm_prog_end(prog);
      float ms = 0.f;
      if (rc == FDM_OK) rc = time_prog(prog, 2, 4, s, &ms);
      HIPCK(hipStreamSynchronize(s));
      fdm_prog_destroy(prog);
      FCK(rc);
      if (ms < *best) *best = ms;
    }
    return FDM_OK;
  };
  bool any = !runner_up.empty();
  for (auto& kv : tuned) any = any || kv.second != 0;
  std::map<std::string, int> keep;
  if (any) {
    float t_h = 0.f, t_t = 0.f;
    FCK(chain_time({}, &t_h));
    FCK(chain_time(tuned, &t_t));
    for (auto& kv : runner_up) {
      std::map<std::string, int> trial = tuned;
      trial[kv.first] = kv.second;
      float t_a = 0.f;
      FCK(chain_time(trial, &t_a));
      if (t_a < 0.997f * t_t) { tuned = trial; t_t = t_a; }
    }
    if (t_t < 0.99f * t_h) {
      float t_h2 = 0.f;
      FCK(chain_time({}, &t_h2));
      t_h = std::min(t_h, t_h2);
    }
    if (t_t < 0.99f * t_h) keep = tuned;
    if (getenv("FDM_TUNE_VERBOSE")) {
      std::string desc;
      for (auto& kv : tuned) desc += kv.first + "=" + std::to_string(kv.second) + ",";
      fprintf(stderr, "[fdm tune] rows=%d candidates: %s chain %.3f -> %.3f ms: %s\n", P->R, desc.c_str(), t_h / 4, t_t / 4, keep.empty() ? "rejected" : "kept");
    }
  }
  P->tiles = keep;
  apply_tile_override(P->tiles);
  P->tile_cache[key] = P->tiles;
  return FDM_OK;
}

}

bool fdm::needs_tune(fdm_plan* P, const std::string& key) {
  return !P->tile_cache.count(key) && tuning_on(P) && P->steps_seen.count(key) && P->steps_seen[key] >= 2000 && !P->tune_failed_shapes.count(key);
}

int fdm::tune_tiles(fdm_plan* P, int force, void* stream) {
  const std::string key = shape_key(P);
  if (P->tile_cache.count(key) || !tuning_on(P)) return FDM_OK;
  if (!force && !needs_tune(P, key)) return FDM_OK;
  const std::map<std::string, int> before = P->tiles;
  const int rc = tune_tiles_impl(P, stream);
  if (rc != FDM_OK) { P->tiles = before; (void)drop_programs(P, stream); if (!force) P->tune_failed_shapes.insert(key); }
  else { store_save(P, P->tiles); P->tune_failed_shapes.erase(key); }
  return rc;
}

void fdm::tune_soft(fdm_plan* P, void* stream) {
  if (tune_tiles(P, 0, stream) != FDM_OK) ++P->tune_failed;
}

void fdm::select_tiles(fdm_plan* P) {
  const std::string key = shape_key(P);
  auto it = P->tile_cache.find(key);
  std::map<std::string, int> want;
  if (it != P->tile_cache.end()) {
    want = it->second;
  } else if (tuning_on(P) && store_lookup(P, want)) {
    apply_tile_override(want);
    P->tile_cache[key] = want;
  } else {
    want.clear();
    apply_tile_override(want);
  }
  P->tiles = want;
}
```

### face-diffusion-model_amd/fdm_amd/_lib.py

```python
import ctypes as C
import os

_HERE = os.path.dirname(os.path.abspath(__file__))
LIB_PATH = os.environ.get("FDM_LIB_PATH") or os.path.join(_HERE, "libfdm_hip.so")

F32, BF16, F16X3, F16 = 0, 1, 2, 3
DTYPE_NAMES = {"f32": F32, "bf16": BF16, "f16x3": F16X3, "f16": F16}
SAMPLER_DPMPP_2M, SAMPLER_DDIM = 0, 1
SLOT_IDLE, SLOT_RUNNING, SLOT_FINISHED = 0, 1, 2
SAMPLER_NAMES = {"dpmpp2m": SAMPLER_DPMPP_2M, "ddim_eta": SAMPLER_DDIM}
ACT_NONE, ACT_RELU, ACT_MISH, ACT_GELU_ERF, ACT_GELU_TANH, ACT_LEAKY02 = range(6)

vp, ll, ci, cf = C.c_void_p, C.c_longlong, C.c_int, C.c_float


class SchedArgs(C.Structure):
    _fields_ = [("x0", vp), ("x0u", vp), ("cfg_scale", cf), ("x", vp), ("x_out", vp),
                ("n", ll), ("n_per_clip", ll), ("tseq", vp), ("step", vp), ("advance", ci),
                ("c1", vp), ("c2", vp), ("sigma", vp), ("sra", vp), ("srm1", vp),
                ("sqrt_an", vp), ("c_n", vp), ("noise", vp), ("noise_stride", ll), ("x_out_t", vp), ("out_dtype", ci), ("arrive", vp),
                ("seed", C.c_ulonglong), ("clip0", ci),
                ("mode", ci), ("x_out_t_lo_off", ll), ("seed_dev", vp),
                ("lm_a", vp), ("lm_b", vp), ("lm_c", vp), ("lm_s", vp), ("x0_hist", vp)]


class GemmArgs(C.Structure):
    _fields_ = [("A", vp), ("lda", ll), ("a_batch_stride", ll),
                ("W", vp), ("ldw", ll), ("w_batch_stride", ll),
                ("M", ci), ("N", ci), ("K", ci), ("batch", ci), ("dtype", ci),
                ("bias", vp), ("bias_batch_stride", ll), ("act", ci),
                ("resid", vp), ("ldr", ll), ("resid_row_mod", ci),
                ("out_f32", vp), ("ldo_f32", ll), ("out_t", vp), ("ldo_t", ll),
                ("out_batch_stride", ll),
                ("out_kp", vp), ("kp_col0", ci), ("out_vp", vp), ("vp_col0", ci),
                ("kv_L", ci), ("kv_Lpad", ci), ("kv_hd", ci),
                ("stat_out", vp), ("ln_stat_in", vp), ("ln_nparts", ci), ("ln_dim", ci), ("ln_eps", cf),
                ("ln_colsum", vp), ("rln_gamma", vp), ("rln_beta", vp), ("incr_counter", vp), ("incr_table", vp), ("tile", ci),
                ("sched_fuse", ci), ("sched", SchedArgs),
                ("a_lo_off", ll), ("w_lo_off", ll), ("out_t_lo_off", ll), ("kv_lo_off", ll),
                ("ksplit", ci), ("ksplit_stride", ll), ("batch2", ci), ("a_batch_stride2", ll), ("out_batch_stride2", ll)]


TILE_AUTO, TILE_64x64, TILE_128x64, TILE_128x128, TILE_64x64_S2, TILE_32x64_S3, TILE_256x128_PP, TILE_80x128, TILE_64x128 = 0, 1, 2, 3, 8, 9, 10, 11, 12
TILE_96x128, TILE_256x128, TILE_64x64_S3, TILE_128x64_S3 = 4, 5, 6, 7


class ModelDesc(C.Structure):
    _fields_ = [(n, ci) for n in ("d", "n_head", "n_layers", "ffn", "G", "c", "n_style", "n_emo", "audio_in", "pair",
                                  "pe_periodic", "period", "latent_mish", "style_mish", "max_len")]


class SampleArgs(C.Structure):
    _fields_ = [("kind", ci), ("x_T", vp), ("out", vp), ("t_list", vp), ("n_steps", ci), ("ddim_steps", ci), ("noise", vp),
                ("seed", C.c_ulonglong), ("clip0", ci), ("cfg_scale", cf), ("eager", ci), ("record", vp), ("graph_steps", ci),
                ("lm_tables", vp)]


class VqDesc(C.Structure):
    _fields_ = [(n, ci) for n in ("G", "c", "K", "n_books", "V3", "pre")]


class AttnArgs(C.Structure):
    _fields_ = [("Q", vp), ("ldq", ll), ("Kp", vp), ("Vp", vp), ("Lpad", ci),
                ("O", vp), ("ldo", ll), ("B", ci), ("H", ci), ("L", ci), ("hd", ci), ("dtype", ci),
                ("scale", cf), ("causal", ci), ("slopes", vp), ("period", ci), ("o_split", ci), ("o_lo_off", ll), ("q_lo_off", ll), ("kv_lo_off", ll),
                ("lens", vp)]


class LnArgs(C.Structure):
    _fields_ = [("x", vp), ("M", ci), ("d", ci), ("add_mat", vp), ("add_tab", vp),
                ("tab_index", vp), ("tab_step", vp), ("gamma", vp), ("beta", vp), ("eps", cf),
                ("act", ci), ("y_f32", vp), ("y_t", vp), ("dtype", ci), ("gamma2", vp), ("beta2", vp), ("y_t_lo_off", ll),
                ("add_mat_L", ci), ("add_mat_group", ci), ("add_mat_wrap", ci), ("x_planes", ci), ("x_plane_stride", ll),
                ("clip_step", vp), ("clip_step_stride", ci), ("clip_rows", ci), ("clip_wrap", ci)]


class SlotGroupArgs(C.Structure):
    _fields_ = [("member", vp), ("frames", vp), ("entries", vp), ("groups", vp), ("x_long", vp), ("hist_long", vp),
                ("arena_frames", ci), ("n_entries", ci), ("n_groups", ci), ("L", ci), ("d", ci), ("frame0", ci), ("frame1", ci),
                ("plain", ci), ("init", ci)]


class SlotBankArgs(C.Structure):
    _fields_ = [("req", vp), ("desc", vp), ("t", vp), ("coef", vp), ("n_samplers", ci), ("n_t", ci), ("n_coef", ci), ("reserved", ci)]


class Pcm(C.Structure):
    _fields_ = [("data", vp), ("format", ci), ("channels", ci), ("rate", ci), ("frames", ll)]


class FlameModelDesc(C.Structure):
    _fields_ = [("V", ci), ("J", ci), ("NB", ci), ("expr_at", ci), ("v_template", vp), ("shapedirs", vp), ("posedirs", vp),
                ("j_regressor", vp), ("parents", vp), ("lbs_weights", vp)]


PCM_S16, PCM_S32, PCM_U8, PCM_F32 = range(4)
MESH_INTERLEAVED, MESH_F16, MESH_NORMALS = 1, 2, 4
WRAP_OFFSETS = 1

STRUCTS = {"fdm_sched_args": SchedArgs, "fdm_gemm_args": GemmArgs, "fdm_attn_args": AttnArgs, "fdm_ln_args": LnArgs,
           "fdm_model_desc": ModelDesc, "fdm_sample_args": SampleArgs, "fdm_vq_desc": VqDesc, "fdm_slot_group_args": SlotGroupArgs,
           "fdm_slot_bank_args": SlotBankArgs, "fdm_pcm": Pcm, "fdm_flame_model": FlameModelDesc}

SYMBOLS = {
    "fdm_last_error": (C.c_char_p, []),
    "fdm_version": (ci, []),
    "fdm_abi_struct_size": (ci, [C.c_char_p]),
    "fdm_device_ok": (ci, []),
    "fdm_op_gemm": (ci, [C.POINTER(GemmArgs), vp]),
    "fdm_gemm_heuristic_tile": (ci, [C.POINTER(GemmArgs)]),
    "fdm_op_attention": (ci, [C.POINTER(AttnArgs), vp]),
    "fdm_op_pack_kv": (ci, [vp, ll, vp, ll, vp, vp, ci, ci, ci, ci, ci, ci, vp]),
    "fdm_op_layernorm": (ci, [C.POINTER(LnArgs), vp]),
    "fdm_op_sched_step": (ci, [C.POINTER(SchedArgs), vp]),
    "fdm_op_slot_sched": (ci, [C.POINTER(SchedArgs), vp, vp, ci, vp]),
    "fdm_op_slot_group_sched": (ci, [C.POINTER(SchedArgs), vp, vp, ci, C.POINTER(SlotGroupArgs), vp]),
    "fdm_op_slot_sched_bank": (ci, [C.POINTER(SchedArgs), vp, vp, ci, C.POINTER(SlotBankArgs), vp]),
    "fdm_op_slot_group_sched_bank": (ci, [C.POINTER(SchedArgs), vp, vp, ci, C.POINTER(SlotGroupArgs), C.POINTER(SlotBankArgs), vp]),
    "fdm_op_cast": (ci, [vp, vp, ll, ci, vp]),
    "fdm_op_vertex_err": (ci, [vp, vp, vp, ci, ci, ci, vp, vp, vp, vp]),
    "fdm_op_motion_std": (ci, [vp, vp, vp, ci, ci, ci, vp, vp, vp]),
    "fdm_op_linear_interp": (ci, [vp, vp, ci, ci, ci, ci, vp]),
    "fdm_op_bias_act": (ci, [vp, vp, vp, ll, ci, ci, vp]),
    "fdm_op_add_rows": (ci, [vp, ci, ci, vp, ci, ci, vp, ci, ci, vp, ll, ci, vp]),
    "fdm_op_small_linear": (ci, [vp, vp, vp, vp, ci, ci, ci, ci, vp]),
    "fdm_op_pad_rows": (ci, [vp, vp, ci, ci, ci, ci, ci, ci, vp]),
    "fdm_op_pad_rows_lens": (ci, [vp, vp, ci, ci, ci, ci, ci, vp, vp]),
    "fdm_op_zero_pad_rows": (ci, [vp, ci, ci, ci, vp, vp]),
    "fdm_op_group_pad": (ci, [vp, vp, ci, ci, ci, ci, ci, ci, vp]),
    "fdm_op_set_ints": (ci, [vp, vp, ci, vp]),
    "fdm_op_mask_samples": (ci, [vp, vp, ci, ci, vp, vp]),
    "fdm_op_group_pad_lens": (ci, [vp, vp, ci, ci, ci, ci, ci, ci, vp, vp]),
    "fdm_op_conv0": (ci, [vp, vp, vp, vp, ci, ci, ci, vp]),
    "fdm_op_conv0_ln_gelu": (ci, [vp, vp, vp, vp, vp, vp, ll, ci, ci, ci, cf, ci, vp]),
    "fdm_op_leaky_instnorm": (ci, [vp, vp, vp, ci, ci, ci, cf, ci, vp]),
    "fdm_op_leaky_instnorm_lens": (ci, [vp, vp, vp, ci, ci, ci, cf, ci, vp, vp]),
    "fdm_op_adain": (ci, [vp, vp, vp, ci, ci, ci, cf, vp]),
    "fdm_op_mean_diff": (ci, [vp, vp, vp, vp, ll, ci, vp]),
    "fdm_op_time_groupnorm": (ci, [vp, vp, vp, vp, vp, ll, ci, ci, ci, cf, ci, ci, vp, ll, vp]),
    "fdm_op_time_groupnorm_lens": (ci, [vp, vp, vp, vp, vp, ll, ci, ci, ci, cf, ci, ci, vp, ll, vp, vp]),
    "fdm_op_vq_quant": (ci, [vp, vp, vp, ci, ci, ci, ci, vp, vp, vp]),
    "fdm_op_vq_stats": (ci, [vp, vp, vp, vp, ci, ci, ci, ci, cf, vp, vp, vp, vp, vp]),
    "fdm_prog_create": (ci, [C.POINTER(vp)]),
    "fdm_prog_destroy": (ci, [vp]),
    "fdm_prog_begin": (ci, [vp]),
    "fdm_prog_end": (ci, [vp]),
    "fdm_prog_run": (ci, [vp, vp]),
    "fdm_prog_instantiate": (ci, [vp, vp]),
    "fdm_prog_replay": (ci, [vp, ci, vp]),
    "fdm_prog_num_ops": (ci, [vp]),
    "fdm_model_preset": (ci, [C.c_char_p, C.POINTER(ModelDesc)]),
    "fdm_plan_create": (ci, [C.POINTER(ModelDesc), ci, ci, ci, ci, C.POINTER(vp)]),
    "fdm_plan_reserve": (ci, [vp, ci, ci, ci]),
    "fdm_plan_destroy": (ci, [vp]),
    "fdm_plan_set_weights": (ci, [vp, C.c_char_p, vp, ll, vp]),
    "fdm_plan_commit": (ci, [vp, vp]),
    "fdm_audio_prepare": (ci, [vp, vp, ci, ci, ci, vp, vp, ci, ci, vp]),
    "fdm_audio_prepare_conds": (ci, [vp, vp, ci, ci, ci, ci, vp, vp, ci, ci, vp]),
    "fdm_denoise_step": (ci, [vp, vp, ci, cf, vp, vp, vp]),
    "fdm_sample_graph": (ci, [vp, C.POINTER(SampleArgs), vp]),
    "fdm_window_layout_host": (ci, [ci, ci, ci, vp, ci]),
    "fdm_window_weights_host": (ci, [ci, ci, ci, vp]),
    "fdm_audio_prepare_windows": (ci, [vp, vp, ci, ci, ci, vp, vp, ci, ci, ci, ci, vp]),
    "fdm_sample_windows": (ci, [vp, C.POINTER(SampleArgs), vp]),
    "fdm_slots_open": (ci, [vp, ci, ci, ci, C.POINTER(SampleArgs), vp]),
    "fdm_slot_admit": (ci, [vp, ci, vp, ci, ci, vp, vp, ci, vp, C.c_ulonglong, ci, vp]),
    "fdm_slots_run": (ci, [vp, ci, vp]),
    "fdm_slot_state": (ci, [vp, ci, C.POINTER(ci), C.POINTER(ci), C.POINTER(ci)]),
    "fdm_slot_read": (ci, [vp, ci, vp, vp]),
    "fdm_slot_peek": (ci, [vp, ci, vp, vp]),
    "fdm_slot_admit_long": (ci, [vp, vp, ci, vp, ci, ci, vp, vp, ci, ci, vp, C.c_ulonglong, ci, vp]),
    "fdm_slot_group": (ci, [vp, ci, C.POINTER(ci), C.POINTER(ci), C.POINTER(ci)]),
    "fdm_slot_read_long": (ci, [vp, ci, vp, vp]),
    "fdm_slot_group_table_host": (ci, [ci, ci, ci, vp, ci, vp, vp, vp, vp, ci]),
    "fdm_slot_sampler_add": (ci, [vp, C.POINTER(SampleArgs), vp]),
    "fdm_slot_sampler_drop": (ci, [vp, ci]),
    "fdm_slot_sampler_info": (ci, [vp, ci, C.POINTER(ci), C.POINTER(ci)]),
    "fdm_slot_admit_as": (ci, [vp, ci, vp, ci, ci, vp, vp, ci, vp, C.c_ulonglong, ci, ci, cf, vp]),
    "fdm_slot_admit_long_as": (ci, [vp, vp, ci, vp, ci, ci, vp, vp, ci, ci, vp, C.c_ulonglong, ci, ci, cf, vp]),
    "fdm_op_cond_rows": (ci, [vp, vp, vp, vp, vp, vp, vp, vp, ll, ci, ci, ci, ci, ci, ci, ci, ci, vp]),
    "fdm_audio_prepare_tracks": (ci, [vp, vp, ci, ci, ci, vp, vp, ci, ci, vp]),
    "fdm_audio_prepare_windows_tracks": (ci, [vp, vp, ci, ci, ci, vp, vp, ci, ci, ci, ci, vp]),
    "fdm_slot_admit_tracks": (ci, [vp, ci, vp, ci, ci, vp, vp, ci, vp, C.c_ulonglong, ci, ci, cf, vp]),
    "fdm_slot_admit_long_tracks": (ci, [vp, vp, ci, vp, ci, ci, vp, vp, ci, ci, vp, C.c_ulonglong, ci, ci, cf, vp]),
    "fdm_window_peek": (ci, [vp, vp, vp]),
    "fdm_op_argmax_rows": (ci, [vp, vp, ll, ci, ci, ci, vp]),
    "fdm_op_vq_quant_rows": (ci, [vp, vp, vp, ci, ci, ci, ci, ci, vp, vp, vp]),
    "fdm_op_vq_stats_rows": (ci, [vp, vp, vp, ci, vp, ci, ci, ci, ci, cf, vp, vp, vp, vp, vp]),
    "fdm_vq_quant_tracks": (ci, [vp, vp, vp, ci, ci, vp, vp, vp]),
    "fdm_vq_quant_stats_tracks": (ci, [vp, vp, vp, vp, ci, ci, cf, vp, vp, vp]),
    "fdm_plan_tune": (ci, [vp, vp]),
    "fdm_plan_get": (ci, [vp, C.c_char_p, C.POINTER(ll)]),
    "fdm_plan_set": (ci, [vp, C.c_char_p, ll]),
    "fdm_hubert_create": (ci, [ci, ci, ci, C.POINTER(vp)]),
    "fdm_hubert_set_weights": (ci, [vp, C.c_char_p, vp, ll, vp]),
    "fdm_hubert_forward": (ci, [vp, vp, ci, ci, ci, ci, ci, vp, C.POINTER(ci), vp]),
    "fdm_hubert_frames": (ci, [ci]),
    "fdm_hubert_forward_ragged": (ci, [vp, vp, vp, ci, ci, vp, vp, vp]),
    "fdm_hubert_destroy": (ci, [vp]),
    "fdm_frontend_create": (ci, [vp, ci, C.POINTER(vp)]),
    "fdm_frontend_samples": (ci, [C.POINTER(Pcm), ci, C.POINTER(ll)]),
    "fdm_frontend_forward": (ci, [vp, C.POINTER(Pcm), ci, ci, ci, vp, ll, vp, vp]),
    "fdm_frontend_destroy": (ci, [vp]),
    "fdm_mesh_adjacency_host": (ci, [vp, ci, ci, vp, vp]),
    "fdm_mesh_create": (ci, [vp, ci, ci, C.POINTER(vp)]),
    "fdm_mesh_frames": (ci, [ci, C.c_double, C.c_double, C.POINTER(ci)]),
    "fdm_mesh_forward": (ci, [vp, vp, vp, ci, ci, vp, ci, C.c_double, C.c_double, ci, vp, vp, ci, vp, vp]),
    "fdm_mesh_destroy": (ci, [vp]),
    "fdm_rig_gram_host": (ci, [vp, vp, ci, ci, C.c_double, vp, vp]),
    "fdm_rig_create": (ci, [vp, ci, ci, vp, C.c_double, vp, vp, ci, C.POINTER(vp)]),
    "fdm_rig_forward": (ci, [vp, vp, vp, ci, ci, C.c_double, C.c_double, vp, vp, ci, vp, vp]),
    "fdm_rig_destroy": (ci, [vp]),
    "fdm_rig_temporal_tables_host": (ci, [vp, ci, C.c_double, vp, vp, vp]),
    "fdm_rig_set_temporal": (ci, [vp, C.c_double, vp]),
    "fdm_flame_tables_host": (ci, [C.POINTER(FlameModelDesc), vp, vp, vp]),
    "fdm_flame_create": (ci, [C.POINTER(FlameModelDesc), vp, vp, ci, C.POINTER(vp)]),
    "fdm_flame_forward": (ci, [vp, vp, ci, ci, vp, ci, vp, vp, vp, vp, ci, ci, vp, vp, vp, vp, vp]),
    "fdm_flame_destroy": (ci, [vp]),
    "fdm_wrap_coords_host": (ci, [vp, vp, ci, ci, vp, ci, vp, vp, vp]),
    "fdm_wrap_create": (ci, [vp, vp, ci, ci, vp, ci, vp, vp, C.POINTER(vp)]),
    "fdm_wrap_binding": (ci, [vp, vp, vp, vp]),
    "fdm_wrap_forward": (ci, [vp, vp, vp, ci, ci, vp, ci, ci, vp, vp]),
    "fdm_wrap_destroy": (ci, [vp]),
    "fdm_render_create": (ci, [vp, ci, ci, ci, ci, vp, vp, vp, vp, ci, cf, vp, vp, C.POINTER(vp)]),
    "fdm_render_set_view": (ci, [vp, vp, vp, vp, vp, ci, cf]),
    "fdm_render_set": (ci, [vp, C.c_char_p, ll]),
    "fdm_render_sample_pattern_host": (ci, [ci, vp]),
    "fdm_render_forward": (ci, [vp, vp, vp, ci, ci, vp, ci, C.c_double, C.c_double, vp, vp, vp, vp, ci, vp, vp]),
    "fdm_render_destroy": (ci, [vp]),
    "fdm_vq_create": (ci, [C.POINTER(VqDesc), ci, C.POINTER(vp)]),
    "fdm_vq_set_weights": (ci, [vp, C.c_char_p, vp, ll, vp]),
    "fdm_vq_quant": (ci, [vp, vp, vp, ci, ci, vp, vp, vp]),
    "fdm_vq_quant_stats": (ci, [vp, vp, vp, vp, ci, ci, cf, vp, vp, vp]),
    "fdm_vq_decode": (ci, [vp, vp, ci, ci, vp, vp]),
    "fdm_vq_decode_ragged": (ci, [vp, vp, vp, ci, ci, vp, vp]),
    "fdm_vq_encode": (ci, [vp, vp, vp, ci, ci, vp, vp]),
    "fdm_vq_destroy": (ci, [vp]),
    "fdm_schedule_host": (ci, [ci, vp]),
    "fdm_ddim_schedule_host": (ci, [ci, ci, vp, vp, vp, vp]),
    "fdm_sampler_tables_host": (ci, [ci, ci, ci, C.c_double, vp, vp, vp, vp, vp]),
    "fdm_alibi_slopes_host": (ci, [ci, vp]),
    "fdm_pe_table_host": (ci, [ci, ci, ci, ci, vp]),
    "fdm_resample_ratio_host": (ci, [ci, C.POINTER(ci), C.POINTER(ci)]),
    "fdm_resample_len_host": (ll, [ci, ll]),
    "fdm_resample_taps_host": (ci, [ci, ci, vp]),
}

_lib = None
LIB_VERSION = 105


class FdmError(RuntimeError):
    pass


def lib():
    global _lib
    if _lib is None:
        if not os.path.exists(LIB_PATH):
            raise FdmError(f"{LIB_PATH} not found: build it with `python -c 'import __graft_entry__ as g; g.build()'` "
                           "(there is no CPU fallback for the product path)")
        l = C.CDLL(LIB_PATH)
        for name, (res, args) in SYMBOLS.items():
            fn = getattr(l, name)
            fn.restype = res
            fn.argtypes = args
        if l.fdm_version() != LIB_VERSION:
            raise FdmError(f"{LIB_PATH}: fdm_version() = {l.fdm_version()}, this binding is for {LIB_VERSION}: rebuild the library "
                           "(python -c 'import __graft_entry__ as g; g.build()')")
        for cname, mirror in STRUCTS.items():
            n = l.fdm_abi_struct_size(cname.encode())
            if n != C.sizeof(mirror):
                raise FdmError(f"{LIB_PATH}: sizeof({cname}) = {n} in the library, {C.sizeof(mirror)} in fdm_amd/_lib.py: rebuild the "
                               "library (python -c 'import __graft_entry__ as g; g.build()') or update the binding")
# ... 10 lines not shown
```

### face-diffusion-model_amd/fdm_amd/denoiser.py

```python
import ctypes as C

import torch

from . import presets, schedule
from ._lib import F32, FdmError, ModelDesc, SampleArgs, check, lib

TILE_SITES = ("enc", "qkv", "qkv_ln", "out", "out_ln", "ffn1", "ffn2", "ffn2_stat", "dec", "dec_ln")


def _dev(t, device):
    return t.detach().to(device=device, dtype=torch.float32).contiguous()


def _stream():
    return torch.cuda.current_stream().cuda_stream


def model_desc(p):
    return ModelDesc(p.d, p.n_head, p.n_layers, p.ffn, p.G, p.c, p.n_style, p.n_emo, p.audio_in, p.pair,
                     1 if p.pe == "periodic" else 0, p.period, int(p.latent_mish), int(p.style_mish), p.max_len)


def window_starts(L_total, window, overlap=60):
    n = lib().fdm_window_layout_host(int(L_total), int(window), int(overlap), None, 0)
    if n < 0:
        check(n)
    buf = (C.c_int * n)()
    check(0 if lib().fdm_window_layout_host(int(L_total), int(window), int(overlap), buf, n) == n else -1)
    return list(buf)


def window_weights(L_total, window, overlap=60):
    n = lib().fdm_window_weights_host(int(L_total), int(window), int(overlap), None)
    if n < 0:
        check(n)
    w = torch.empty(n, min(int(window), int(L_total)), dtype=torch.float32)
    check(0 if lib().fdm_window_weights_host(int(L_total), int(window), int(overlap), C.c_void_p(w.data_ptr())) == n else -1)
    return w


class DenoiserPlan:
    def __init__(self, preset, weights, dtype=F32, device="cuda:0"):
        self.p = presets.get(preset)
        self.dtype = dtype
        self.device = torch.device(device)
        if self.device.type != "cuda":
            raise FdmError("DenoiserPlan runs on the HIP path only (no CPU fallback)")
        self.h = None
        self.B = self.L = self.M = 0
        self.S = 1
        self.cfg = False
        self._keep, self._inputs = [], None
        h = C.c_void_p()
        desc = model_desc(self.p)
        with torch.cuda.device(self.device):
            check(lib().fdm_plan_create(C.byref(desc), 1, 1, 0, dtype, C.byref(h)))
            self.h = h
            buf = schedule.make_buffers(1000)
            c1, c2, sg = schedule.ddpm_tables(buf)
            tabs = {"sched.c1": c1, "sched.c2": c2, "sched.sigma": sg, "sched.sra": buf["sqrt_recip_alphas_cumprod"],
                    "sched.srm1": buf["sqrt_recipm1_alphas_cumprod"],
                    "PE.pe": schedule.positional_table(self.p.d, self.p.pe, self.p.period, self.p.max_len + 30)}
            keep = []
            for k, v in list(weights.items()) + list(tabs.items()):
                if k.startswith("audio_encoder.") or (k == "PE.pe" and v is not tabs["PE.pe"]):
                    continue
                t = v.detach().to(torch.float32).contiguous()
                keep.append(t)
                check(lib().fdm_plan_set_weights(h, k.encode(), t.data_ptr(), t.numel(), _stream()))
            torch.cuda.current_stream().synchronize()
            check(lib().fdm_plan_commit(h, _stream()))

    def __del__(self):
        try:
            if self.h:
                lib().fdm_plan_destroy(self.h)
                self.h = None
        except Exception:
            pass

    def _track(self, what, n, B, L, vec, track):
        if track is not None:
            t = torch.as_tensor(track)
            t = t.unsqueeze(0).expand(B, -1, -1) if t.dim() == 2 else t
            if t.dim() != 3 or t.shape[0] != B or t.shape[1] < L or t.shape[2] != n:
                raise FdmError(f"{what} track has shape {tuple(torch.as_tensor(track).shape)}, expected [{B}, >= {L}, {n}] (or [>= {L}, {n}])")
            return _dev(t[:, :L], self.device)
        if vec is None:
            raise FdmError(f"this preset needs a {what} vector or a {what} track")
        v = _dev(vec, self.device)
# ... 303 lines not shown

    def admit_long(self, slots, hub, style=None, emo=None, x_T=None, L_total=None, overlap=60, seed=0, clip_id=0, sampler=0, cfg_scale=None,
                   style_track=None, emotion_track=None):
        p, dv = self.p, self.device
        hub = _dev(hub, dv).reshape(-1, hub.shape[-1])
        N, fw = hub.shape
        L_total = N // p.pair if L_total is None else int(L_total)
        x = _dev(x_T, dv).reshape(-1)
        if x.numel() != L_total * p.d:
            raise FdmError(f"x_T has {x.numel()} elements, expected L_total*G*c = {L_total * p.d}")
        ids = (C.c_int * len(slots))(*[int(s) for s in slots])
        if style_track is not None or emotion_track is not None:
            st, et = self._tracks(1, L_total, None if style is None else torch.as_tensor(style).reshape(-1),
                                  None if emo is None else torch.as_tensor(emo).reshape(-1), style_track, emotion_track)
            scale = self._slot_scale if cfg_scale is None else float(cfg_scale)
            with torch.cuda.device(dv):
                check(lib().fdm_slot_admit_long_tracks(self.h, C.cast(ids, C.c_void_p), len(slots), hub.data_ptr(), N, fw, st.data_ptr(),
                                                       et.data_ptr() if et is not None else None, L_total, int(overlap), x.data_ptr(),
                                                       int(seed), int(clip_id), int(sampler), scale, _stream()))
            self._slot_inputs[int(slots[0])] = (hub, st, et, x)
            return L_total
        style = _dev(style, dv).reshape(-1)
        emo = _dev(emo, dv).reshape(-1) if (p.n_emo and emo is not None) else None
        with torch.cuda.device(dv):
            if sampler == 0 and cfg_scale is None:
                check(lib().fdm_slot_admit_long(self.h, C.cast(ids, C.c_void_p), len(slots), hub.data_ptr(), N, fw, style.data_ptr(),
                                                emo.data_ptr() if emo is not None else None, L_total, int(overlap), x.data_ptr(),
                                                int(seed), int(clip_id), _stream()))
            else:
                scale = self._slot_scale if cfg_scale is None else float(cfg_scale)
                check(lib().fdm_slot_admit_long_as(self.h, C.cast(ids, C.c_void_p), len(slots), hub.data_ptr(), N, fw, style.data_ptr(),
                                                   emo.data_ptr() if emo is not None else None, L_total, int(overlap), x.data_ptr(),
                                                   int(seed), int(clip_id), int(sampler), scale, _stream()))
        self._slot_inputs[int(slots[0])] = (hub, style, emo, x)
        return L_total

    def slot_group(self, slot):
        a, n, lt = C.c_int(), C.c_int(), C.c_int()
        check(lib().fdm_slot_group(self.h, int(slot), C.byref(a), C.byref(n), C.byref(lt)))
        return a.value, n.value, lt.value

    def read_long(self, leader):
        L_total = self.slot_group(leader)[2]
        out = torch.empty(1, max(L_total, 1) * self.p.G, self.p.c, device=self.device)
        with torch.cuda.device(self.device):
            check(lib().fdm_slot_read_long(self.h, int(leader), out.data_ptr(), _stream()))
        return out

    def run(self, n_steps):
        with torch.cuda.device(self.device):
            check(lib().fdm_slots_run(self.h, int(n_steps), _stream()))

    def slot_state(self, slot):
        d, t, st = C.c_int(), C.c_int(), C.c_int()
        check(lib().fdm_slot_state(self.h, int(slot), C.byref(d), C.byref(t), C.byref(st)))
        return d.value, t.value, st.value

    def read_slot(self, slot, L):
        out = torch.empty(1, int(L) * self.p.G, self.p.c, device=self.device)
        with torch.cuda.device(self.device):
            check(lib().fdm_slot_read(self.h, int(slot), out.data_ptr(), _stream()))
        return out

    def peek_slot(self, slot):
        out = torch.empty(1, self.L * self.p.G, self.p.c, device=self.device)
        with torch.cuda.device(self.device):
            check(lib().fdm_slot_peek(self.h, int(slot), out.data_ptr(), _stream()))
        return out

    def tune(self):
        with torch.cuda.device(self.device):
            check(lib().fdm_plan_tune(self.h, _stream()))

    def get(self, key):
        v = C.c_longlong()
        check(lib().fdm_plan_get(self.h, key.encode(), C.byref(v)))
        return v.value

    def set(self, key, value):
        check(lib().fdm_plan_set(self.h, key.encode(), int(value)))

    @property
    def tiles(self):
        return {k: self.get("tile." + k) for k in TILE_SITES}

    @property
    def fuse_ln3(self):
        return bool(self.get("fuse_ln3"))
```

### face-diffusion-model_amd/fdm_amd/ops.py

```python
import ctypes as C

import torch

from . import _lib
from ._lib import (ACT_GELU_ERF, ACT_GELU_TANH, ACT_LEAKY02, ACT_MISH, ACT_NONE, ACT_RELU, BF16, F16, F16X3, F32,
                   AttnArgs, GemmArgs, LnArgs, SchedArgs, check, lib)


class Split:

    def __init__(self, planes, code, row0=0, col0=0):
        self.planes, self.code, self.row0, self.col0 = planes, code, row0, col0
        self.lo_off = planes[0].numel()

    @classmethod
    def empty(cls, rows, cols, code, device):
        return cls(torch.zeros(2, rows, cols, device=device, dtype=tdtype(code)), code)

    def __getitem__(self, sl):
        if not isinstance(sl, slice) or sl.stop is not None or sl.step is not None:
            raise _lib.FdmError("Split operands support [r0:] row offsets only")
        return Split(self.planes, self.code, self.row0 + (sl.start or 0), self.col0)

    @property
# ... 21 lines not shown

def _p(t):
    if t is None:
        return None
    if not t.is_cuda:
        raise _lib.FdmError("fdm_amd ops need device tensors (no CPU fallback on the product path)")
    return t.data_ptr()


def _lo(t):
    return t.lo_off if isinstance(t, Split) else 0


def stream():
    return torch.cuda.current_stream().cuda_stream


def tdtype(code):
    return {BF16: torch.bfloat16, F16X3: torch.float16, F16: torch.float16}.get(code, torch.float32)


def is_split(code):
    return code == F16X3


def code_of(t):
    if isinstance(t, Split):
        return t.code
    if t.dtype == torch.bfloat16:
        return BF16
    if t.dtype == torch.float32:
        return F32
    if t.dtype == torch.float16:
        return F16
    raise _lib.FdmError(f"unsupported dtype {t.dtype}")


def gemm(A, W, M, N, K, *, lda=None, ldw=None, bias=None, act=ACT_NONE, resid=None, ldr=None, resid_row_mod=0,
         out_f32=None, ldo_f32=None, out_t=None, ldo_t=None, batch=1, a_bs=0, w_bs=0, bias_bs=0, out_bs=0,
         out_kp=None, kp_col0=0, out_vp=None, vp_col0=0, kv_L=0, kv_Lpad=0, kv_hd=0,
         stat_out=None, ln_stat_in=None, ln_nparts=0, ln_dim=0, ln_eps=1e-5, ln_colsum=None, rln_gamma=None, rln_beta=None,
         incr_counter=None, incr_table=None, tile=0, sched=None, ksplit=0, ksplit_stride=0,
         batch2=0, a_bs2=0, out_bs2=0):
    a = GemmArgs()
    a.A, a.lda, a.a_batch_stride = _p(A), lda if lda is not None else K, a_bs
    a.W, a.ldw, a.w_batch_stride = _p(W), ldw if ldw is not None else K, w_bs
    a.M, a.N, a.K, a.batch, a.dtype = M, N, K, batch, code_of(A)
    if code_of(W) != a.dtype:
        raise _lib.FdmError("gemm: A and W operand kinds differ")
    a.a_lo_off, a.w_lo_off, a.out_t_lo_off = _lo(A), _lo(W), _lo(out_t)
    a.kv_lo_off = _lo(out_kp) or _lo(out_vp)
    a.bias, a.bias_batch_stride, a.act = _p(bias), bias_bs, act
    a.resid, a.ldr, a.resid_row_mod = _p(resid), (ldr if ldr is not None else N), resid_row_mod
    a.out_f32, a.ldo_f32 = _p(out_f32), (ldo_f32 if ldo_f32 is not None else N)
    a.out_t, a.ldo_t = _p(out_t), (ldo_t if ldo_t is not None else N)
    a.out_batch_stride = out_bs
    a.out_kp, a.kp_col0, a.out_vp, a.vp_col0 = _p(out_kp), kp_col0, _p(out_vp), vp_col0
    a.kv_L, a.kv_Lpad, a.kv_hd = kv_L, kv_Lpad, kv_hd
    a.stat_out, a.ln_stat_in, a.ln_nparts, a.ln_dim, a.ln_eps = _p(stat_out), _p(ln_stat_in), ln_nparts, ln_dim, ln_eps
    a.ln_colsum, a.rln_gamma, a.rln_beta = _p(ln_colsum), _p(rln_gamma), _p(rln_beta)
    a.incr_counter, a.incr_table = _p(incr_counter), _p(incr_table)
    a.tile = tile
    a.batch2, a.a_batch_stride2, a.out_batch_stride2 = batch2, a_bs2, out_bs2
    a.ksplit, a.ksplit_stride = ksplit, ksplit_stride
    if sched is not None:
        a.sched_fuse, a.sched = 1, sched
    check(lib().fdm_op_gemm(C.byref(a), stream()))


def kv_pad(L):
    return (L + 31) // 32 * 32


def kv_buffers(B, H, L, hd, dtype, device):
    Lpad = kv_pad(L)
    return (torch.zeros(B * H, Lpad * hd, device=device, dtype=dtype),
            torch.zeros(B * H, Lpad * hd, device=device, dtype=dtype), Lpad)


def pack_kv(K, V, Kp, Vp, *, B, H, L, Lpad, hd, ldk, ldv):
    check(lib().fdm_op_pack_kv(_p(K), ldk, _p(V), ldv, _p(Kp), _p(Vp), B, H, L, Lpad, hd, code_of(K), stream()))


def attention(Q, Kp, Vp, O, *, B, H, L, hd, ldq, ldo, Lpad, scale, causal=False, slopes=None, period=1, lens=None):
    a = AttnArgs()
    a.Q, a.ldq, a.Kp, a.Vp, a.Lpad = _p(Q), ldq, _p(Kp), _p(Vp), Lpad
    a.O, a.ldo, a.B, a.H, a.L, a.hd, a.dtype = _p(O), ldo, B, H, L, hd, code_of(Q)
    if isinstance(Q, Split):
        a.q_lo_off, a.kv_lo_off, a.o_lo_off = Q.lo_off, Kp.lo_off, O.lo_off
    elif isinstance(O, Split):
        a.o_split, a.o_lo_off = O.code, O.lo_off
    a.scale, a.causal, a.slopes, a.period, a.lens = scale, int(causal), _p(slopes), period, _p(lens)
    check(lib().fdm_op_attention(C.byref(a), stream()))


def layernorm(x, gamma, beta, M, d, *, add_mat=None, add_tab=None, tab_index=None, tab_step=None, eps=1e-5,
              act=ACT_NONE, y_f32=None, y_t=None, dtype=F32, gamma2=None, beta2=None, x_planes=0, x_plane_stride=0,
              clip_step=None, clip_step_stride=1, clip_rows=0, clip_wrap=0, add_mat_group=0, add_mat_wrap=0, add_mat_L=0):
    a = LnArgs()
    a.x, a.M, a.d, a.add_mat, a.add_tab = _p(x), M, d, _p(add_mat), _p(add_tab)
    a.tab_index, a.tab_step, a.gamma, a.beta, a.eps = _p(tab_index), _p(tab_step), _p(gamma), _p(beta), eps
    a.act, a.y_f32, a.y_t, a.dtype = act, _p(y_f32), _p(y_t), dtype
    a.gamma2, a.beta2, a.y_t_lo_off = _p(gamma2), _p(beta2), _lo(y_t)
    a.x_planes, a.x_plane_stride = x_planes, x_plane_stride
    a.add_mat_group, a.add_mat_wrap, a.add_mat_L = add_mat_group, add_mat_wrap, add_mat_L
    if clip_step is not None:
        a.clip_step, a.clip_step_stride, a.clip_rows, a.clip_wrap = _p(clip_step), clip_step_stride, clip_rows, clip_wrap
    check(lib().fdm_op_layernorm(C.byref(a), stream()))


def sched_args(mode, x0, x, x_out, n, *, x0u=None, cfg_scale=0.0, n_per_clip=0, tseq=None, step=None, advance=0,
               c1=None, c2=None, sigma=None, sra=None, srm1=None, sqrt_an=None, c_n=None, noise=None, noise_stride=0,
               seed=0, clip0=0, x_out_t=None, arrive=None, lm_a=None, lm_b=None, lm_c=None, lm_s=None, x0_hist=None, seed_dev=None):
    a = SchedArgs()
    a.x0, a.x0u, a.cfg_scale, a.x, a.x_out = _p(x0), _p(x0u), cfg_scale, _p(x), _p(x_out)
    a.n, a.n_per_clip, a.tseq, a.step, a.advance = n, n_per_clip, _p(tseq), _p(step), advance
    a.c1, a.c2, a.sigma, a.sra, a.srm1 = _p(c1), _p(c2), _p(sigma), _p(sra), _p(srm1)
    a.sqrt_an, a.c_n, a.noise, a.noise_stride = _p(sqrt_an), _p(c_n), _p(noise), noise_stride
    a.seed, a.clip0, a.mode = seed, clip0, mode
    a.x_out_t, a.out_dtype, a.arrive = _p(x_out_t), (code_of(x_out_t) if x_out_t is not None else 0), _p(arrive)
    a.x_out_t_lo_off = _lo(x_out_t)
    a.lm_a, a.lm_b, a.lm_c, a.lm_s, a.x0_hist = _p(lm_a), _p(lm_b), _p(lm_c), _p(lm_s), _p(x0_hist)
    if seed_dev is not None:
        a.seed_dev = _p(seed_dev)
    return a


def sched_step(mode, x0, x, x_out, n, **kw):
    a = sched_args(mode, x0, x, x_out, n, **kw)
    check(lib().fdm_op_sched_step(C.byref(a), stream()))


def slot_sched(mode, x0, x, x_out, n, state, keys, n_slots, **kw):
    a = sched_args(mode, x0, x, x_out, n, **kw)
    check(lib().fdm_op_slot_sched(C.byref(a), _p(state), _p(keys), n_slots, stream()))


def slot_group_sched(mode, x0, x, x_out, n, state, keys, n_slots, *, member, frames, entries, groups, x_long, hist_long=None, L, d,
                     frame0=0, frame1=None, plain=1, init=0, **kw):
    a = sched_args(mode, x0, x, x_out, n, **kw)
    g = _lib.SlotGroupArgs()
    g.member, g.frames, g.entries, g.groups, g.x_long, g.hist_long = _p(member), _p(frames), _p(entries), _p(groups), _p(x_long), _p(hist_long)
    g.arena_frames, g.n_entries, g.n_groups, g.L, g.d = frames.shape[0], entries.shape[0], groups.shape[0], L, d
    g.frame0, g.frame1, g.plain, g.init = frame0, frames.shape[0] if frame1 is None else frame1, plain, init
    check(lib().fdm_op_slot_group_sched(C.byref(a), _p(state), _p(keys), n_slots, C.byref(g), stream()))


def bank_args(req, desc, t, coef):
    b = _lib.SlotBankArgs()
    b.req, b.desc, b.t, b.coef = _p(req), _p(desc), _p(t), _p(coef)
    b.n_samplers, b.n_t, b.n_coef = desc.shape[0], t.numel(), coef.numel()
    return b


def slot_sched_bank(x0, x, x_out, n, state, keys, n_slots, *, req, desc, t, coef, **kw):
    a = sched_args(0, x0, x, x_out, n, **kw)
    b = bank_args(req, desc, t, coef)
    check(lib().fdm_op_slot_sched_bank(C.byref(a), _p(state), _p(keys), n_slots, C.byref(b), stream()))


def slot_group_sched_bank(x0, x, x_out, n, state, keys, n_slots, *, req, desc, t, coef, member, frames, entries, groups, x_long, hist_long=None,
                          L, d, frame0=0, frame1=None, plain=1, init=0, **kw):
    a = sched_args(0, x0, x, x_out, n, **kw)
    g = _lib.SlotGroupArgs()
    g.member, g.frames, g.entries, g.groups, g.x_long, g.hist_long = _p(member), _p(frames), _p(entries), _p(groups), _p(x_long), _p(hist_long)
    g.arena_frames, g.n_entries, g.n_groups, g.L, g.d = frames.shape[0], entries.shape[0], groups.shape[0], L, d
    g.frame0, g.frame1, g.plain, g.init = frame0, frames.shape[0] if frame1 is None else frame1, plain, init
    b = bank_args(req, desc, t, coef)
    check(lib().fdm_op_slot_group_sched_bank(C.byref(a), _p(state), _p(keys), n_slots, C.byref(g), C.byref(b), stream()))


def cast(src, dst):
    check(lib().fdm_op_cast(_p(src), _p(dst), src.numel(), code_of(dst), stream()))


def to_operand(src_f32, dtype):
    if dtype == F32:
        return src_f32
    if is_split(dtype):
        dst = Split(torch.empty((2,) + tuple(src_f32.shape), dtype=tdtype(dtype), device=src_f32.device), dtype)
    else:
        dst = torch.empty(src_f32.shape, dtype=tdtype(dtype), device=src_f32.device)
    cast(src_f32.contiguous(), dst)
    return dst


def bias_act(inp, vec, out, rows, d, act):
    check(lib().fdm_op_bias_act(_p(inp), _p(vec), _p(out), rows, d, act, stream()))
# ... 191 lines not shown
```

### include/fdm_hip.h

```cpp
#ifndef FDM_HIP_H
#define FDM_HIP_H

#ifdef __cplusplus
extern "C" {
#endif

#define FDM_F32 0
#define FDM_BF16 1
#define FDM_F16X3 2
#define FDM_F16 3

#define FDM_ACT_NONE 0
#define FDM_ACT_RELU 1
#define FDM_ACT_MISH 2
#define FDM_ACT_GELU_ERF 3
#define FDM_ACT_GELU_TANH 4
#define FDM_ACT_LEAKY02 5

#define FDM_OK 0
#define FDM_ERR_ARG (-1)
#define FDM_ERR_SHAPE (-2)
#define FDM_ERR_HIP (-3)
#define FDM_ERR_STATE (-4)

// ... 14 lines not shown
  void* x_out_t; int out_dtype;
  unsigned int* arrive;
  unsigned long long seed; int clip0;
  int mode;
  long long x_out_t_lo_off;
  const unsigned long long* seed_dev;
  const float* lm_a; const float* lm_b; const float* lm_c; const float* lm_s;
  float* x0_hist;
} fdm_sched_args;
int fdm_op_sched_step(const fdm_sched_args* a, void* stream);
int fdm_op_slot_sched(const fdm_sched_args* a, const int* state, const unsigned long long* keys, int n_slots, void* stream);
typedef struct fdm_slot_group_args {
  const int* member; const int* frames; const void* entries; const int* groups;
  float* x_long; float* hist_long;
  int arena_frames, n_entries, n_groups;
  int L, d;
  int frame0, frame1;
  int plain, init;
} fdm_slot_group_args;
int fdm_op_slot_group_sched(const fdm_sched_args* a, const int* state, const unsigned long long* keys, int n_slots,
                            const fdm_slot_group_args* g, void* stream);
typedef struct fdm_slot_bank_args {
  const void* req; const int* desc; const int* t; const float* coef;
  int n_samplers, n_t, n_coef;
  int reserved;
} fdm_slot_bank_args;
int fdm_op_slot_sched_bank(const fdm_sched_args* a, const int* state, const unsigned long long* keys, int n_slots,
                           const fdm_slot_bank_args* b, void* stream);
int fdm_op_slot_group_sched_bank(const fdm_sched_args* a, const int* state, const unsigned long long* keys, int n_slots,
                                 const fdm_slot_group_args* g, const fdm_slot_bank_args* b, void* stream);

typedef struct fdm_gemm_args {
  const void* A; long long lda; long long a_batch_stride;
  const void* W; long long ldw; long long w_batch_stride;
  int M, N, K, batch;
  int dtype;
  const float* bias; long long bias_batch_stride;
  int act;
  const float* resid; long long ldr; int resid_row_mod;
  float* out_f32; long long ldo_f32;
  void* out_t; long long ldo_t;
  long long out_batch_stride;
  void* out_kp; int kp_col0;
  void* out_vp; int vp_col0;
  int kv_L; int kv_Lpad; int kv_hd;
  float* stat_out;
  const float* ln_stat_in; int ln_nparts; int ln_dim; float ln_eps;
  const float* ln_colsum;
  const float* rln_gamma; const float* rln_beta;
  int* incr_counter;
  const int* incr_table;
  int tile;
  int sched_fuse;
  fdm_sched_args sched;
  long long a_lo_off, w_lo_off, out_t_lo_off;
  long long kv_lo_off;
  int ksplit; long long ksplit_stride;
  int batch2; long long a_batch_stride2, out_batch_stride2;
} fdm_gemm_args;
#define FDM_TILE_AUTO 0
#define FDM_TILE_64x64 1
#define FDM_TILE_128x64 2
#define FDM_TILE_128x128 3
#define FDM_TILE_64x64_S2 8
#define FDM_TILE_32x64_S3 9
#define FDM_TILE_256x128_PP 10
#define FDM_TILE_80x128 11
#define FDM_TILE_64x128 12
#define FDM_TILE_96x128 4
#define FDM_TILE_256x128 5
#define FDM_TILE_64x64_S3 6
#define FDM_TILE_128x64_S3 7
#define FDM_TILE_MAX 12
#define FDM_TILE_GENERAL 0x100
#define FDM_TILE_LOCKSTEP 0x200
#define FDM_TILE_ID_MASK 0xff
int fdm_op_gemm(const fdm_gemm_args* a, void* stream);
int fdm_gemm_heuristic_tile(const fdm_gemm_args* a);

typedef struct fdm_attn_args {
  const void* Q; long long ldq;
  const void* Kp;
  const void* Vp; int Lpad;
  void* O; long long ldo;
  int B, H, L, hd;
  int dtype;
  float scale;
  int causal;
  const float* slopes;
  int period;
  int o_split; long long o_lo_off;
  long long q_lo_off, kv_lo_off;
  const int* lens;
} fdm_attn_args;
int fdm_op_attention(const fdm_attn_args* a, void* stream);
int fdm_op_pack_kv(const void* K, long long ldk, const void* V, long long ldv, void* Kp, void* Vp,
                   int B, int H, int L, int Lpad, int hd, int dtype, void* stream);

typedef struct fdm_ln_args {
  const float* x; int M, d;
  const float* add_mat;
  const float* add_tab;
  const int* tab_index; const int* tab_step;
  const float* gamma; const float* beta; float eps;
  int act;
  float* y_f32; void* y_t; int dtype;
  const float* gamma2; const float* beta2;
  long long y_t_lo_off;
  int add_mat_L, add_mat_group, add_mat_wrap;
  int x_planes; long long x_plane_stride;
  const int* clip_step; int clip_step_stride, clip_rows, clip_wrap;
} fdm_ln_args;
int fdm_op_layernorm(const fdm_ln_args* a, void* stream);


int fdm_op_cast(const float* src, void* dst, long long n, int dtype, void* stream);
int fdm_op_bias_act(const float* in, const float* vec, float* out, long long rows, int d, int act, void* stream);
int fdm_op_add_rows(const float* a, int a_div, int a_mod, const float* b, int b_div, int b_mod,
                    const float* c, int c_div, int c_mod, float* out, long long M, int d, void* stream);
int fdm_op_small_linear(const float* x, const float* W, const float* bias, float* out, int B, int K, int d,
                        int act, void* stream);
int fdm_op_cond_rows(const float* pe, const float* style, const float* emo, const float* sw, const float* sb, const float* ew,
                     const float* eb, float* out, long long uncond_off, int B, int L, int L_clip, int L_track, int d, int n_style,
                     int n_emo, int act, void* stream);
int fdm_op_pad_rows(const void* in, void* out, int B, int L, int d, int pad, int dtype, int zero, void* stream);
int fdm_op_pad_rows_lens(const void* in, void* out, int B, int L, int d, int pad, int dtype, const int* lens, void* stream);
int fdm_op_zero_pad_rows(float* x, int B, int L, int d, const int* lens, void* stream);
int fdm_op_set_ints(int* dst, const int* src, int n, void* stream);
int fdm_op_mask_samples(const float* wav, float* out, int B, int n, const int* lens, void* stream);
int fdm_op_group_pad_lens(const void* in, void* out, int B, int T, int d, int groups, int pad, int dtype, const int* lens, void* stream);
int fdm_op_conv0(const float* wav, const float* w, const float* bias, float* out, int B, int n, int T0, void* stream);
int fdm_op_conv0_ln_gelu(const float* wav, const float* w, const float* bias, const float* gamma, const float* beta, void* out,
                         long long out_lo_off, int B, int n, int T0, float eps, int dtype, void* stream);
int fdm_op_leaky_instnorm(const float* x, float* y_f32, void* y_t, int B, int L, int d, float eps, int dtype, void* stream);
int fdm_op_leaky_instnorm_lens(const float* x, float* y_f32, void* y_t, int B, int L, int d, float eps, int dtype, const int* lens, void* stream);
int fdm_op_time_groupnorm(const float* x, const float* gamma, const float* beta, float* y_f32, void* y_t, long long y_t_lo_off, int B, int T, int C,
                          float eps, int act, int dtype, void* scratch, long long scratch_bytes, void* stream);
int fdm_op_time_groupnorm_lens(const float* x, const float* gamma, const float* beta, float* y_f32, void* y_t, long long y_t_lo_off, int B, int T, int C,
                               float eps, int act, int dtype, void* scratch, long long scratch_bytes, const int* lens, void* stream);
int fdm_op_mean_diff(const float* a, const float* b, float* partial, float* out, long long n, int l1, void* stream);
int fdm_op_vertex_err(const float* gt, const float* pred, const int* region, int R, int F, int V,
                      float* frame_max, double* frame_sum, double* out, void* stream);
int fdm_op_motion_std(const float* verts, const float* tmpl, const int* region, int R, int F, int V,
                      double* partial, double* out, void* stream);
int fdm_op_linear_interp(const float* x, float* y, int B, int Tin, int Tout, int C, void* stream);
int fdm_op_adain(const float* content, const float* style, float* out, int NC, int Lc, int Ls, float eps, void* stream);
int fdm_op_group_pad(const void* in, void* out, int B, int T, int d, int groups, int pad, int dtype, void* stream);

int fdm_op_vq_quant(const float* z, const float* codebook, const int* book, int B, int R, int c, int K,
                    float* zq_bcl, long long* idx, void* stream);
int fdm_op_vq_stats(const float* z, const float* codebook, const int* book, const long long* idx, int B, int R, int c, int K, float beta,
                    float* min_encodings, double* partial, int* hist, float* out, void* stream);
int fdm_op_argmax_rows(const float* x, int* book, long long rows, int n, int rep, int n_books, void* stream);
int fdm_op_vq_quant_rows(const float* z, const float* codebook, const int* book_rows, int n_books, int B, int R, int c, int K,
                         float* zq_bcl, long long* idx, void* stream);
int fdm_op_vq_stats_rows(const float* z, const float* codebook, const int* book_rows, int n_books, const long long* idx, int B, int R, int c,
                         int K, float beta, float* min_encodings, double* partial, int* hist, float* out, void* stream);

typedef struct fdm_prog fdm_prog;
int fdm_prog_create(fdm_prog** out);
int fdm_prog_destroy(fdm_prog* p);
int fdm_prog_begin(fdm_prog* p);
int fdm_prog_end(fdm_prog* p);
int fdm_prog_run(fdm_prog* p, void* stream);
int fdm_prog_instantiate(fdm_prog* p, void* stream);
int fdm_prog_replay(fdm_prog* p, int n, void* stream);
int fdm_prog_num_ops(fdm_prog* p);

typedef struct fdm_model_desc {
  int d, n_head, n_layers, ffn;
  int G, c;
  int n_style, n_emo;
  int audio_in, pair;
  int pe_periodic, period;
  int latent_mish, style_mish;
  int max_len;
} fdm_model_desc;
int fdm_model_preset(const char* name, fdm_model_desc* out);

typedef struct fdm_plan fdm_plan;
int fdm_plan_create(const fdm_model_desc* desc, int B, int L, int cfg, int dtype, fdm_plan** out);
int fdm_plan_reserve(fdm_plan* p, int B, int L, int cfg);
int fdm_plan_destroy(fdm_plan* p);
int fdm_plan_set_weights(fdm_plan* p, const char* name, const float* ptr, long long n, void* stream);
int fdm_plan_commit(fdm_plan* p, void* stream);
int fdm_audio_prepare(fdm_plan* p, const float* hub, int B, int N, int fw, const float* style, const float* emo,
                      int L, int cfg, void* stream);
int fdm_audio_prepare_conds(fdm_plan* p, const float* hub, int B, int N, int fw, int S, const float* style, const float* emo,
                            int L, int cfg, void* stream);
int fdm_denoise_step(fdm_plan* p, const float* x_t, int t, float cfg_scale, float* x0_hat, float* x0_uncond, void* stream);
typedef struct fdm_sample_args {
  int kind;
  const float* x_T; float* out;
  const int* t_list; int n_steps;
  int ddim_steps;
  const float* noise;
  unsigned long long seed; int clip0;
  float cfg_scale;
  int eager;
  float* record;
  int graph_steps;
  const float* lm_tables;
} fdm_sample_args;
int fdm_sample_graph(fdm_plan* p, const fdm_sample_args* a, void* stream);
int fdm_window_layout_host(int L_total, int window, int overlap, int* starts, int cap);
int fdm_window_weights_host(int L_total, int window, int overlap, float* w);
int fdm_audio_prepare_windows(fdm_plan* p, const float* hub, int B, int N, int fw, const float* style, const float* emo,
                              int L_total, int window, int overlap, int cfg, void* stream);
int fdm_sample_windows(fdm_plan* p, const fdm_sample_args* a, void* stream);
int fdm_window_peek(fdm_plan* p, float* out, void* stream);
#define FDM_SLOT_IDLE 0
#define FDM_SLOT_RUNNING 1
#define FDM_SLOT_FINISHED 2
int fdm_slots_open(fdm_plan* p, int B, int L, int cfg, const fdm_sample_args* sampler, void* stream);
int fdm_slot_admit(fdm_plan* p, int slot, const float* hub, int N, int fw, const float* style, const float* emo, int L_clip,
                   const float* x_T, unsigned long long seed, int clip_id, void* stream);
int fdm_slots_run(fdm_plan* p, int n_steps, void* stream);
int fdm_slot_state(fdm_plan* p, int slot, int* steps_done, int* steps_total, int* status);
int fdm_slot_read(fdm_plan* p, int slot, float* out, void* stream);
int fdm_slot_peek(fdm_plan* p, int slot, float* out, void* stream);
int fdm_slot_admit_long(fdm_plan* p, const int* slots, int n, const float* hub, int N, int fw, const float* style, const float* emo,
                        int L_total, int overlap, const float* x_T, unsigned long long seed, int clip_id, void* stream);
int fdm_slot_group(fdm_plan* p, int slot, int* leader, int* n, int* L_total);
int fdm_slot_read_long(fdm_plan* p, int leader, float* out, void* stream);
int fdm_slot_group_table_host(int L_total, int L, int overlap, const int* slots, int n, int* off, int* ent_slot, int* ent_start,
                              float* ent_wt, int cap);
int fdm_slot_sampler_add(fdm_plan* p, const fdm_sample_args* sampler, void* stream);
int fdm_slot_sampler_drop(fdm_plan* p, int id);
int fdm_slot_sampler_info(fdm_plan* p, int id, int* kind, int* n_steps);
int fdm_slot_admit_as(fdm_plan* p, int slot, const float* hub, int N, int fw, const float* style, const float* emo, int L_clip,
                      const float* x_T, unsigned long long seed, int clip_id, int sampler, float cfg_scale, void* stream);
int fdm_slot_admit_long_as(fdm_plan* p, const int* slots, int n, const float* hub, int N, int fw, const float* style, const float* emo,
                           int L_total, int overlap, const float* x_T, unsigned long long seed, int clip_id, int sampler, float cfg_scale,
                           void* stream);
int fdm_audio_prepare_tracks(fdm_plan* p, const float* hub, int B, int N, int fw, const float* style, const float* emo, int L, int cfg,
                             void* stream);
int fdm_audio_prepare_windows_tracks(fdm_plan* p, const float* hub, int B, int N, int fw, const float* style, const float* emo,
                                     int L_total, int window, int overlap, int cfg, void* stream);
int fdm_slot_admit_tracks(fdm_plan* p, int slot, const float* hub, int N, int fw, const float* style, const float* emo, int L_clip,
                          const float* x_T, unsigned long long seed, int clip_id, int sampler, float cfg_scale, void* stream);
int fdm_slot_admit_long_tracks(fdm_plan* p, const int* slots, int n, const float* hub, int N, int fw, const float* style, const float* emo,
                               int L_total, int overlap, const float* x_T, unsigned long long seed, int clip_id, int sampler,
                               float cfg_scale, void* stream);
int fdm_plan_tune(fdm_plan* p, void* stream);
int fdm_plan_get(fdm_plan* p, const char* key, long long* out);
int fdm_plan_set(fdm_plan* p, const char* key, long long value);

typedef struct fdm_audio_encoder fdm_audio_encoder;
int fdm_hubert_create(int kind, int n_layers, int dtype, fdm_audio_encoder** out);
int fdm_hubert_set_weights(fdm_audio_encoder* e, const char* name, const float* ptr, long long n, void* stream);
int fdm_hubert_forward(fdm_audio_encoder* e, const float* wav, int B, int n_samples, int frame_num, int interp_in_fps, int interp_out_fps,
                       float* out, int* n_frames, void* stream);
int fdm_hubert_frames(int n_samples);
int fdm_hubert_forward_ragged(fdm_audio_encoder* e, const float* wav, const int* n_samples, int B, int n_max, float* out, int* n_frames, void* stream);
int fdm_hubert_destroy(fdm_audio_encoder* e);

#define FDM_PCM_S16 0
#define FDM_PCM_S32 1
#define FDM_PCM_U8 2
#define FDM_PCM_F32 3
typedef struct fdm_pcm { const void* data; int format; int channels; int rate; long long frames; } fdm_pcm;
typedef struct fdm_frontend fdm_frontend;
int fdm_frontend_create(const int* rates, int n_rates, fdm_frontend** out);
int fdm_frontend_samples(const fdm_pcm* clip, int pad, long long* n);
int fdm_frontend_forward(fdm_frontend* f, const fdm_pcm* clips, int B, int pad, int normalize, float* wav, long long n_max, int* n_samples,
                         void* stream);
int fdm_frontend_destroy(fdm_frontend* f);

typedef struct fdm_vq_desc { int G, c, K, n_books, V3, pre; } fdm_vq_desc;
typedef struct fdm_vq fdm_vq;
int fdm_vq_create(const fdm_vq_desc* desc, int dtype, fdm_vq** out);
int fdm_vq_set_weights(fdm_vq* v, const char* name, const float* ptr, long long n, void* stream);
int fdm_vq_quant(fdm_vq* v, const float* z, const float* emo_one_hot, int B, int R, float* zq_bcl, long long* idx, void* stream);
int fdm_vq_quant_stats(fdm_vq* v, const float* z, const float* emo_one_hot, const long long* idx, int B, int R, float beta,
                       float* min_encodings, float* out2, void* stream);
int fdm_vq_quant_tracks(fdm_vq* v, const float* z, const float* emo, int B, int R, float* zq_bcl, long long* idx, void* stream);
int fdm_vq_quant_stats_tracks(fdm_vq* v, const float* z, const float* emo, const long long* idx, int B, int R, float beta,
                              float* min_encodings, float* out2, void* stream);
int fdm_vq_decode(fdm_vq* v, const float* zq_bcl, int B, int R, float* out, void* stream);
int fdm_vq_decode_ragged(fdm_vq* v, const float* zq_bcl, const int* frames, int B, int R_max, float* out, void* stream);
int fdm_vq_encode(fdm_vq* v, const float* x, const float* emo_one_hot, int B, int L, float* latent, void* stream);
int fdm_vq_destroy(fdm_vq* v);

#define FDM_MESH_INTERLEAVED 1
#define FDM_MESH_F16 2
#define FDM_MESH_NORMALS 4
typedef struct fdm_mesh fdm_mesh;
int fdm_mesh_adjacency_host(const int* faces, int F, int V, int* offsets, int* items);
int fdm_mesh_create(const int* faces, int F, int V, fdm_mesh** out);
int fdm_mesh_frames(int frames_in, double fps_in, double fps_out, int* frames_out);
int fdm_mesh_forward(fdm_mesh* m, const float* offsets, const int* frames, int B, int L_max, const float* tmpl, int tmpl_rows, double fps_in,
                     double fps_out, int flags, void* pos, void* nrm, int L_out_max, int* frames_out, void* stream);
int fdm_mesh_destroy(fdm_mesh* m);

typedef struct fdm_rig fdm_rig;
int fdm_rig_gram_host(const float* basis, const float* vweight, int K, int V, double ridge, double* gram, float* chol);
int fdm_rig_create(const float* basis, int K, int V, const float* vweight, double ridge, const float* lo, const float* hi, int sweeps,
                   fdm_rig** out);
int fdm_rig_forward(fdm_rig* r, const float* offsets, const int* frames, int B, int L_max, double fps_in, double fps_out, float* coef,
                    float* proj, int L_out_max, int* frames_out, void* stream);
int fdm_rig_destroy(fdm_rig* r);
int fdm_rig_temporal_tables_host(const double* gram, int K, double smooth, const float* sweights, double* lam, double* Q);
int fdm_rig_set_temporal(fdm_rig* r, double smooth, const float* sweights);

typedef struct fdm_flame_model {
  int V, J, NB, expr_at;
  const float* v_template; const float* shapedirs; const float* posedirs; const float* j_regressor;
  const int* parents; const float* lbs_weights;
} fdm_flame_model;
typedef struct fdm_flame fdm_flame;
int fdm_flame_tables_host(const fdm_flame_model* m, float* D, float* JT, float* JD);
int fdm_flame_create(const fdm_flame_model* m, const int* lmk_verts, const float* lmk_bary, int NL, fdm_flame** out);
int fdm_flame_forward(fdm_flame* f, const float* shape, int NS, int shape_rows, const float* expr, int NE, const float* pose, const float* transl,
                      const float* extra, const int* frames, int B, int L_max, float* verts, float* lmk, float* xforms, float* posefeat,
                      void* stream);
int fdm_flame_destroy(fdm_flame* f);

#define FDM_WRAP_OFFSETS 1
typedef struct fdm_wrap fdm_wrap;
int fdm_wrap_coords_host(const float* src_rest, const int* faces, int F, int V, const float* dst_rest, int Vt, const int* face_idx,
                         float* uvh , float* dist );
int fdm_wrap_create(const float* src_rest, const int* faces, int F, int V, const float* dst_rest, int Vt,
                    const int* face_idx , const float* weights , fdm_wrap** out);
int fdm_wrap_binding(const fdm_wrap* w, int* face_idx, float* uvh, float* dist);
int fdm_wrap_forward(fdm_wrap* w, const float* offsets, const int* frames, int B, int L_max, const float* tmpl, int tmpl_rows, int flags,
                     float* out, void* stream);
int fdm_wrap_destroy(fdm_wrap* w);
// ... 29 lines not shown
```

Before: 1981 frames/s.

## Add autotuned launch shapes for attention query split and multi-row layernorm

Adds a qs field to attention arguments so the two-sub-tile query kernel can be forced or disabled regardless of sequence length. Adds a multi-row layernorm variant that packs 2 or 4 rows per block, sharing one launch and reducing the number of small blocks. The tuner now times these shapes per site and adopts one only when it beats the incumbent, and pins and validation are threaded through plan_set and the cache. This adds API and struct-layout changes, and tuning time.

```diff
diff --git a/face-diffusion-model_amd/csrc/attention.hpp b/face-diffusion-model_amd/csrc/attention.hpp
--- a/face-diffusion-model_amd/csrc/attention.hpp
+++ b/face-diffusion-model_amd/csrc/attention.hpp
@@ -268,7 +268,7 @@
   constexpr int qs2 = 384;
   const int groups = (a.B * a.H + 7) / 8 * 8;
   if constexpr (HD <= 128 && Opnd<T>::NP == 1) {
-    if (a.L >= qs2) {
+    if (a.qs == 2 || (a.qs == 0 && a.L >= qs2)) {
       dim3 grid((a.L + 31) / 32 * groups);
       if (a.lens) { hipLaunchKernelGGL((attn_kernel<T, HD, 2, true>), grid, dim3(256), 0, s, ATTN_PRELOAD_ARGS, a); return; }
       hipLaunchKernelGGL((attn_kernel<T, HD, 2>), grid, dim3(256), 0, s, ATTN_PRELOAD_ARGS, a);
diff --git a/face-diffusion-model_amd/csrc/elementwise.hpp b/face-diffusion-model_amd/csrc/elementwise.hpp
--- a/face-diffusion-model_amd/csrc/elementwise.hpp
+++ b/face-diffusion-model_amd/csrc/elementwise.hpp
@@ -7,18 +7,21 @@
 
 namespace fdm {
 
-template <typename T, int NV, bool HEAVY, bool CLIP = false>
-__global__ __launch_bounds__(64 * NV) void ln_row_kernel(const float* p_x, const float* p_add_mat, const float* p_add_tab, const int* p_tab_step,
+template <typename T, int NV, bool HEAVY, bool CLIP = false, int RW = 1>
+__global__ __launch_bounds__(64 * NV * RW) void ln_row_kernel(const float* p_x, const float* p_add_mat, const float* p_add_tab, const int* p_tab_step,
                                                          const int* p_tab_index, int p_add_mat_group, int p_add_mat_wrap, int p_add_mat_L,
                                                          const fdm_ln_args p) {
-  __shared__ float red[4][NV];
+  __shared__ float red[RW][4][NV];
   constexpr int d = 256 * NV;
 #ifdef FDM_GEMM_STAMPS
   const unsigned long long t_first = wall_clock64();
   unsigned long long t_loaded = 0, t_reduced = 0;
 #endif
-  const int tid = threadIdx.x, lane = tid & 63, wave = tid >> 6;
-  const int row = blockIdx.x, col = tid * 4;
+  const int sub = RW == 1 ? 0 : __builtin_amdgcn_readfirstlane((int)threadIdx.x / (64 * NV));
+  const int tid = RW == 1 ? (int)threadIdx.x : (int)threadIdx.x - sub * (64 * NV), lane = tid & 63, wave = tid >> 6;
+  const int row_w = RW == 1 ? (int)blockIdx.x : (int)blockIdx.x * RW + sub;
+  const bool live = RW == 1 || row_w < p.M;
+  const int row = live ? row_w : p.M - 1, col = tid * 4;
   const bool two = p.gamma2 != nullptr;
   const f32x4 zero = f32x4{0.f, 0.f, 0.f, 0.f};
   f32x4 v = *(const f32x4*)(p_x + (size_t)row * d + col);
@@ -51,11 +54,11 @@
   const f32x4 e = p_add_tab ? em + et : em;
   auto block_sum = [&](float x, int slot) {
     x = wave_sum(x);
-    if (lane == 0) red[slot][wave] = x;
+    if (lane == 0) red[sub][slot][wave] = x;
     __syncthreads();
     float t = 0.f;
 #pragma unroll
-    for (int w = 0; w < NV; ++w) t += red[slot][w];
+    for (int w = 0; w < NV; ++w) t += red[sub][slot][w];
     return t;
   };
 #pragma unroll
@@ -94,8 +97,8 @@
 #pragma unroll
     for (int j = 0; j < 4; ++j) y[j] = fmaxf(y[j], 0.f);
   }
-  if (p.y_f32) st16(p.y_f32 + (size_t)row * d + col, y);
-  if (p.y_t) store_opnd4<T>((typename Opnd<T>::E*)p.y_t + (size_t)row * d + col, p.y_t_lo_off, y);
+  if (live && p.y_f32) st16(p.y_f32 + (size_t)row * d + col, y);
+  if (live && p.y_t) store_opnd4<T>((typename Opnd<T>::E*)p.y_t + (size_t)row * d + col, p.y_t_lo_off, y);
 #ifdef FDM_GEMM_STAMPS
   if (p.x_planes == 0 && p.x_plane_stride) {
     const unsigned long long t_issued = wall_clock64();
@@ -110,9 +113,25 @@
 }
 
 #define LN_PRELOAD_ARGS a.x, a.add_mat, a.add_tab, a.tab_step, a.tab_index, a.add_mat_group, a.add_mat_wrap, a.add_mat_L
+template <typename T, int RW>
+static hipError_t ln_launch_rows(const fdm_ln_args& a, hipStream_t s) {
+  dim3 grid((a.M + RW - 1) / RW);
+  if (a.clip_step) {
+    if (a.d == 512) hipLaunchKernelGGL((ln_row_kernel<T, 2, false, true, RW>), grid, dim3(128 * RW), 0, s, LN_PRELOAD_ARGS, a);
+    else hipLaunchKernelGGL((ln_row_kernel<T, 4, false, true, RW>), grid, dim3(256 * RW), 0, s, LN_PRELOAD_ARGS, a);
+  } else {
+    if (a.d == 512) hipLaunchKernelGGL((ln_row_kernel<T, 2, false, false, RW>), grid, dim3(128 * RW), 0, s, LN_PRELOAD_ARGS, a);
+    else hipLaunchKernelGGL((ln_row_kernel<T, 4, false, false, RW>), grid, dim3(256 * RW), 0, s, LN_PRELOAD_ARGS, a);
+  }
+  return hipGetLastError();
+}
 template <typename T, bool HEAVY>
 static hipError_t ln_launch_h(const fdm_ln_args& a, hipStream_t s) {
   dim3 grid(a.M);
+  if (a.shape != 0) {
+    if (HEAVY || (a.d != 512 && a.d != 1024) || a.shape < 0 || a.shape > 2) return hipErrorInvalidValue;
+    if constexpr (!HEAVY) return a.shape == 1 ? ln_launch_rows<T, 2>(a, s) : ln_launch_rows<T, 4>(a, s);
+  }
   if constexpr (!HEAVY) {
     if (a.clip_step) {
       switch (a.d) {
diff --git a/face-diffusion-model_amd/csrc/fdm_hip.hip b/face-diffusion-model_amd/csrc/fdm_hip.hip
--- a/face-diffusion-model_amd/csrc/fdm_hip.hip
+++ b/face-diffusion-model_amd/csrc/fdm_hip.hip
@@ -177,7 +177,6 @@
   if (!a) return fail(FDM_ERR_ARG, "gemm_heuristic_tile: null argument");
   fdm_gemm_args b = *a;
   b.tile = 0;
-  if (b.batch2 >= 1 && b.ksplit <= 1 && !b.sched_fuse && gemm_tile_override() > 0) return gemm_tile_override();
   return gemm_requested_tile(b);
 }
 
@@ -199,6 +198,9 @@
   if (a->slopes && a->period <= 0) return fail(FDM_ERR_ARG, "attention: period must be positive");
   if (a->lens && (a->causal || (a->hd != 64 && a->hd != 128)))
     return fail(FDM_ERR_ARG, "attention: per-clip lengths need causal = 0 and head_dim 64 or 128");
+  if (a->qs < 0 || a->qs > 2) return fail(FDM_ERR_ARG, "attention: qs %d outside 0..2", a->qs);
+  if (a->qs == 2 && (a->hd == 256 || a->dtype == FDM_F16X3))
+    return fail(FDM_ERR_ARG, "attention: qs = 2 exists for head_dim 64 / 128 of the single-plane kinds (head_dim %d, dtype %d)", a->hd, a->dtype);
   fdm_attn_args c = *a;
   return submit([c](hipStream_t s) { return fdm::attn_launch(c, s); }, stream, "attention");
 }
@@ -229,6 +231,9 @@
   if (a->clip_step && (a->clip_rows <= 0 || a->clip_step_stride <= 0 || a->clip_wrap < 0 || (a->clip_wrap > 0 && a->clip_wrap % a->clip_rows)))
     return fail(FDM_ERR_SHAPE, "layernorm: clip_step needs clip_rows > 0, clip_step_stride > 0 and clip_rows | clip_wrap (got %d, %d, %d)", a->clip_rows, a->clip_step_stride, a->clip_wrap);
   if (a->clip_step && a->act != FDM_ACT_NONE && a->act != FDM_ACT_RELU) return fail(FDM_ERR_ARG, "layernorm: clip_step runs with FDM_ACT_NONE / FDM_ACT_RELU only");
+  if (a->shape < 0 || a->shape > 2) return fail(FDM_ERR_ARG, "layernorm: shape %d outside 0..2", a->shape);
+  if (a->shape && ((a->d != 512 && a->d != 1024) || (a->act != FDM_ACT_NONE && a->act != FDM_ACT_RELU)))
+    return fail(FDM_ERR_ARG, "layernorm: shape %d exists for d = 512 / 1024 with FDM_ACT_NONE / FDM_ACT_RELU (d %d, act %d)", a->shape, a->d, a->act);
   fdm_ln_args c = *a;
   return submit([c](hipStream_t s) {
     switch (c.dtype) {
diff --git a/face-diffusion-model_amd/csrc/plan.hip b/face-diffusion-model_amd/csrc/plan.hip
--- a/face-diffusion-model_amd/csrc/plan.hip
+++ b/face-diffusion-model_amd/csrc/plan.hip
@@ -78,6 +78,11 @@
 void set_ln_stats(fdm_gemm_args& g, const fdm_plan* P) { g.ln_stat_in = P->stats; g.ln_nparts = P->m.d / 64; g.ln_dim = P->m.d; g.ln_eps = 1e-5f; }
 void set_ksplit(fdm_gemm_args& g, int S, long long plane) { if (S > 1) { g.ksplit = S; g.ksplit_stride = plane; } }
 void set_ksplit(fdm_ln_args& ln, int S, long long plane) { if (S > 1) { ln.x_planes = S; ln.x_plane_stride = plane; } }
+
+int site_shape(const fdm_plan* P, const char* label) {
+  auto it = P->tiles.find(label);
+  return it == P->tiles.end() ? 0 : it->second;
+}
 
 int plan_gemm(fdm_plan* P, const char* label, fdm_gemm_args a, void* stream) {
   if (P->tune_rec) (*P->tune_rec)[label].push_back(a);
@@ -324,6 +329,7 @@
     at.B = BB; at.H = m.n_head; at.L = L; at.hd = P->hd; at.dtype = P->dtype;
     at.scale = 1.0f / std::sqrt((float)P->hd); at.causal = 1; at.slopes = P->slopes; at.period = m.period;
     if (split) { at.q_lo_off = P->q_lo; at.kv_lo_off = P->kv_lo; at.o_lo_off = P->ctx.lo; }
+    at.qs = site_shape(P, "attn");
     FCK(fdm_op_attention(&at, stream));
     FCK(need(P, lname(l, "self_attn.out_proj.bias"), d, &b));
     g = gemm_op(P, P->ctx, P->wt[lname(l, "self_attn.out_proj.weight")], R, d, d);
@@ -348,6 +354,7 @@
     FCK(need(P, lname(l, "norm2.weight"), d, &ln.gamma2)); FCK(need(P, lname(l, "norm2.bias"), d, &ln.beta2));
     ln.y_f32 = P->h2; ln.dtype = P->dtype;
     if (both) { ln.y_t = P->h2t.p; ln.y_t_lo_off = P->h2t.lo; }
+    ln.shape = site_shape(P, "ln12");
     FCK(fdm_op_layernorm(&ln, stream));
     FCK(need(P, lname(l, "linear1.bias"), m.ffn, &b));
     g = gemm_op(P, P->h2t, P->wt[lname(l, "linear1.weight")], R, m.ffn, d);
@@ -368,6 +375,7 @@
       set_ksplit(ln, P->ksplit_ffn2, (long long)R * d);
       FCK(need(P, lname(l, "norm3.weight"), d, &ln.gamma)); FCK(need(P, lname(l, "norm3.bias"), d, &ln.beta));
       if (both) { ln.y_t = P->ht.p; ln.y_t_lo_off = P->ht.lo; }
+      ln.shape = site_shape(P, "ln3");
       FCK(fdm_op_layernorm(&ln, stream));
     }
   }
@@ -403,9 +411,8 @@
 };
 
 std::string tiles_sig(const fdm_plan* P) {
-  std::string s;
-  for (auto& kv : P->tiles)
-    if (kv.second) s += kv.first + "=" + std::to_string(kv.second) + ",";
+  std::string s = tile_set_text(P->tiles);
+  if (!s.empty()) s += ",";
   s += "ks" + std::to_string(P->ksplit_out) + std::to_string(P->ksplit_ffn2) + (P->lockstep ? "L" : "");
   return s;
 }
@@ -1503,6 +1510,8 @@
   else if (k == "graph_launches") *out = P->last_graph_launches;
   else if (k == "fuse_ln3") *out = P->fuse_ln3;
   else if (k == "rows") *out = P->R;
+  else if (k == "attn_qs") *out = P->pin_attn_qs;
+  else if (k == "ln_shape") *out = P->pin_ln_shape;
   else if (k == "ksplit.out") *out = P->ksplit_out;
   else if (k == "ksplit.ffn2") *out = P->ksplit_ffn2;
   else if (k == "tuned") *out = P->tile_cache.count(shape_key(P)) ? 1 : 0;
@@ -1522,8 +1531,19 @@
 }
 
 int fdm_plan_set(fdm_plan* P, const char* key, long long value) {
-  if (!P || !key) return fail(FDM_ERR_ARG, "plan_set: null argument");
+  if (!key) return fail(FDM_ERR_ARG, "plan_set: null argument");
   const std::string k(key);
+  if ((k == "attn_qs" || k == "ln_shape") && (value < 0 || value > 2)) return fail(FDM_ERR_ARG, "plan_set: %s = %lld outside 0..2", key, value);
+  if (!P) return fail(FDM_ERR_ARG, "plan_set: null argument");
+  if (k == "attn_qs" || k == "ln_shape") {
+    if (k == "attn_qs" && value == 2 && !attn_qs2_ok(P)) return fail(FDM_ERR_ARG, "plan_set: attn_qs = 2 needs head_dim 64 / 128 and a single-plane kind");
+    if (k == "ln_shape" && value && !ln_shapes_ok(P)) return fail(FDM_ERR_ARG, "plan_set: ln_shape = %lld needs d = 512 / 1024 (d = %d)", value, P->m.d);
+    int& cur = k == "attn_qs" ? P->pin_attn_qs : P->pin_ln_shape;
+    if (cur == (int)value) return FDM_OK;
+    cur = (int)value;
+    P->tile_cache.clear(); P->tiles.clear(); apply_pins(P, P->tiles);
+    return drop_programs(P, nullptr);
+  }
   if (k == "tune") { P->tune_enabled = value != 0; return FDM_OK; }
   if (k == "tune_lazy") { P->tune_lazy = value != 0; return FDM_OK; }
   if (k == "slot_long_frames" || k == "slot_long_groups") {
@@ -1554,14 +1574,19 @@
     }
     return FDM_OK;
   }
-  if (k == "lockstep") { P->lockstep = value != 0; P->tile_cache.clear(); P->tiles.clear(); return drop_programs(P, nullptr); }
+  if (k == "lockstep") { P->lockstep = value != 0; P->tile_cache.clear(); P->tiles.clear(); apply_pins(P, P->tiles); return drop_programs(P, nullptr); }
   if (k == "untune") {
-    P->tile_cache.clear(); P->steps_seen.clear(); P->tiles.clear(); P->tune_failed_shapes.clear();
+    P->tile_cache.clear(); P->steps_seen.clear(); P->tiles.clear(); P->tune_failed_shapes.clear(); apply_pins(P, P->tiles);
     return drop_programs(P, nullptr);
   }
   if (k.rfind("tile.", 0) == 0) {
     if (value < 0 || value > FDM_TILE_MAX) return fail(FDM_ERR_ARG, "plan_set: unknown tile %lld", value);
-    P->tiles[k.substr(5)] = (int)value;
+    const std::string site = k.substr(5);
+    if (site == "attn" || site == "ln12" || site == "ln3") {
+      if (value > 2 || (site == "attn" ? (value == 2 && !attn_qs2_ok(P)) : (value != 0 && !ln_shapes_ok(P))))
+        return fail(FDM_ERR_ARG, "plan_set: %s = %lld is not a launch shape of this plan", key, value);
+    }
+    P->tiles[site] = (int)value;
     P->tile_cache[shape_key(P)] = P->tiles;
     return drop_programs(P, nullptr);
   }
diff --git a/face-diffusion-model_amd/csrc/plan.hpp b/face-diffusion-model_amd/csrc/plan.hpp
--- a/face-diffusion-model_amd/csrc/plan.hpp
+++ b/face-diffusion-model_amd/csrc/plan.hpp
@@ -51,6 +51,7 @@
   int ksplit_out = 1, ksplit_ffn2 = 1;
   int x1_planes = 0;
   int lockstep = 0;
+  int pin_attn_qs = 0, pin_ln_shape = 0;
   int tune_lazy = 0;
   long long last_graph_launches = 0, launches_per_step = 0;
   int win_n = 0, win_len = 0, win_total = 0, win_overlap = 0, win_B = 0;
@@ -96,4 +97,8 @@
 int tune_tiles(fdm_plan* P, int force, void* stream);
 void tune_soft(fdm_plan* P, void* stream);
 void select_tiles(fdm_plan* P);
+void apply_pins(const fdm_plan* P, std::map<std::string, int>& tiles);
+std::string tile_set_text(const std::map<std::string, int>& tiles);
+bool attn_qs2_ok(const fdm_plan* P);
+bool ln_shapes_ok(const fdm_plan* P);
 }
diff --git a/face-diffusion-model_amd/csrc/tune.hip b/face-diffusion-model_amd/csrc/tune.hip
--- a/face-diffusion-model_amd/csrc/tune.hip
+++ b/face-diffusion-model_amd/csrc/tune.hip
@@ -38,9 +38,20 @@
   return out;
 }
 
-void apply_tile_override(std::map<std::string, int>& tiles) {
+void drop_bad_shapes(const fdm_plan* P, std::map<std::string, int>& tiles) {
+  for (const char* site : {"attn", "ln12", "ln3"}) {
+    auto it = tiles.find(site);
+    if (it == tiles.end()) continue;
+    const bool attn = !strcmp(site, "attn");
+    if (it->second < 0 || it->second > 2 || (attn ? (it->second == 2 && !attn_qs2_ok(P)) : (it->second != 0 && !ln_shapes_ok(P)))) tiles.erase(it);
+  }
+}
+
+void apply_tile_override(const fdm_plan* P, std::map<std::string, int>& tiles) {
   if (const char* ov = getenv("FDM_TILE_OVERRIDE"))
     for (auto& kv : parse_tiles(ov)) tiles[kv.first] = kv.second;
+  drop_bad_shapes(P, tiles);
+  apply_pins(P, tiles);
 }
 
 std::string store_key(const fdm_plan* P) {
@@ -73,16 +84,14 @@
     if (kv.second < 0 || kv.second > FDM_TILE_MAX) return false;
     if (kv.second) tiles[kv.first] = kv.second;
   }
+  drop_bad_shapes(P, tiles);
   return true;
 }
 
 void store_save(const fdm_plan* P, const std::map<std::string, int>& tiles) {
   std::map<std::string, std::string> lines;
   if (!store_read(lines)) return;
-  std::string v;
-  for (auto& kv : tiles)
-    if (kv.second) v += (v.empty() ? "" : ",") + kv.first + "=" + std::to_string(kv.second);
-  lines[store_key(P)] = v;
+  lines[store_key(P)] = tile_set_text(tiles);
   const std::string path = getenv("FDM_TILE_CACHE"), tmp = path + ".tmp" + std::to_string((long long)getpid());
   {
     std::ofstream f(tmp, std::ios::trunc);
@@ -214,12 +223,73 @@
       fprintf(stderr, "[fdm tune] rows=%d candidates: %s chain %.3f -> %.3f ms: %s\n", P->R, desc.c_str(), t_h / 4, t_t / 4, keep.empty() ? "rejected" : "kept");
     }
   }
+  apply_tile_override(P, keep);
+  struct ShapeSite { const char* site; std::vector<int> cands; };
+  std::vector<ShapeSite> sites;
+  const int qs_rule = P->L >= 384 ? 2 : 1;
+  if (attn_qs2_ok(P)) sites.push_back({"attn", {3 - qs_rule}});
+  if (ln_shapes_ok(P)) {
+    sites.push_back({"ln12", {1, 2}});
+    if (!P->fuse_ln3) sites.push_back({"ln3", {1, 2}});
+  }
+  for (const ShapeSite& st : sites) {
+    if (keep.count(st.site)) continue;
+    float t_inc = 0.f, t_best = 1e30f;
+    int best = 0;
+    FCK(chain_time(keep, &t_inc));
+    std::string desc;
+    for (int c : st.cands) {
+      std::map<std::string, int> trial = keep;
+      trial[st.site] = c;
+      float t = 0.f;
+      FCK(chain_time(trial, &t));
+      desc += " " + std::to_string(c) + ":" + std::to_string(t / 4 * 1e3f);
+      if (t < t_best) { t_best = t; best = c; }
+    }
+    if (t_best < 0.99f * t_inc) {
+      float t2 = 0.f;
+      FCK(chain_time(keep, &t2));
+      t_inc = std::min(t_inc, t2);
+    }
+    const bool adopt = t_best < 0.99f * t_inc;
+    if (adopt) keep[st.site] = best;
+    if (getenv("FDM_TUNE_VERBOSE"))
+      fprintf(stderr, "[fdm tune] rows=%d site %s: incumbent %.2f us, candidates (shape:us)%s: %s\n", P->R, st.site, t_inc / 4 * 1e3f, desc.c_str(),
+              adopt ? ("kept " + std::to_string(best)).c_str() : "incumbent kept");
+  }
   P->tiles = keep;
-  apply_tile_override(P->tiles);
   P->tile_cache[key] = P->tiles;
   return FDM_OK;
 }
 
+}
+
+bool fdm::attn_qs2_ok(const fdm_plan* P) { return kind(P->dtype).planes == 1 && P->hd <= 128; }
+bool fdm::ln_shapes_ok(const fdm_plan* P) { return P->m.d == 512 || P->m.d == 1024; }
+
+void fdm::apply_pins(const fdm_plan* P, std::map<std::string, int>& tiles) {
+  if (P->pin_attn_qs) tiles["attn"] = P->pin_attn_qs;
+  if (P->pin_ln_shape) tiles["ln12"] = tiles["ln3"] = P->pin_ln_shape;
+}
+
+std::string fdm::tile_set_text(const std::map<std::string, int>& tiles) {
+  std::string v;
+  for (auto& kv : tiles)
+    if (kv.second) v += (v.empty() ? "" : ",") + kv.first + "=" + std::to_string(kv.second);
+  return v;
+}
+
+extern "C" int fdm_tile_set_text(const char* sites, char* out, int cap) {
+  if (!sites || !out || cap <= 0) return fail(FDM_ERR_ARG, "tile_set_text: null argument");
+  std::map<std::string, int> tiles;
+  for (auto& kv : parse_tiles(sites)) {
+    if (kv.second < 0 || kv.second > FDM_TILE_MAX) return fail(FDM_ERR_ARG, "tile_set_text: %s = %d outside 0..%d", kv.first.c_str(), kv.second, FDM_TILE_MAX);
+    tiles[kv.first] = kv.second;
+  }
+  const std::string v = tile_set_text(tiles);
+  if ((int)v.size() + 1 > cap) return fail(FDM_ERR_ARG, "tile_set_text: %d bytes needed", (int)v.size() + 1);
+  memcpy(out, v.c_str(), v.size() + 1);
+  return (int)v.size();
 }
 
 bool fdm::needs_tune(fdm_plan* P, const std::string& key) {
@@ -248,11 +318,11 @@
   if (it != P->tile_cache.end()) {
     want = it->second;
   } else if (tuning_on(P) && store_lookup(P, want)) {
-    apply_tile_override(want);
+    apply_tile_override(P, want);
     P->tile_cache[key] = want;
   } else {
     want.clear();
-    apply_tile_override(want);
+    apply_tile_override(P, want);
   }
   P->tiles = want;
 }
diff --git a/face-diffusion-model_amd/fdm_amd/_lib.py b/face-diffusion-model_amd/fdm_amd/_lib.py
--- a/face-diffusion-model_amd/fdm_amd/_lib.py
+++ b/face-diffusion-model_amd/fdm_amd/_lib.py
@@ -61,7 +61,7 @@
 
 
 class AttnArgs(C.Structure):
-    _fields_ = [("Q", vp), ("ldq", ll), ("Kp", vp), ("Vp", vp), ("Lpad", ci),
+    _fields_ = [("Q", vp), ("ldq", ll), ("Kp", vp), ("Vp", vp), ("Lpad", ci), ("qs", ci),
                 ("O", vp), ("ldo", ll), ("B", ci), ("H", ci), ("L", ci), ("hd", ci), ("dtype", ci),
                 ("scale", cf), ("causal", ci), ("slopes", vp), ("period", ci), ("o_split", ci), ("o_lo_off", ll), ("q_lo_off", ll), ("kv_lo_off", ll),
                 ("lens", vp)]
@@ -70,7 +70,7 @@
 class LnArgs(C.Structure):
     _fields_ = [("x", vp), ("M", ci), ("d", ci), ("add_mat", vp), ("add_tab", vp),
                 ("tab_index", vp), ("tab_step", vp), ("gamma", vp), ("beta", vp), ("eps", cf),
-                ("act", ci), ("y_f32", vp), ("y_t", vp), ("dtype", ci), ("gamma2", vp), ("beta2", vp), ("y_t_lo_off", ll),
+                ("act", ci), ("y_f32", vp), ("y_t", vp), ("dtype", ci), ("shape", ci), ("gamma2", vp), ("beta2", vp), ("y_t_lo_off", ll),
                 ("add_mat_L", ci), ("add_mat_group", ci), ("add_mat_wrap", ci), ("x_planes", ci), ("x_plane_stride", ll),
                 ("clip_step", vp), ("clip_step_stride", ci), ("clip_rows", ci), ("clip_wrap", ci)]
 
@@ -190,6 +190,7 @@
     "fdm_vq_quant_tracks": (ci, [vp, vp, vp, ci, ci, vp, vp, vp]),
     "fdm_vq_quant_stats_tracks": (ci, [vp, vp, vp, vp, ci, ci, cf, vp, vp, vp]),
     "fdm_plan_tune": (ci, [vp, vp]),
+    "fdm_tile_set_text": (ci, [C.c_char_p, C.c_char_p, ci]),
     "fdm_plan_get": (ci, [vp, C.c_char_p, C.POINTER(ll)]),
     "fdm_plan_set": (ci, [vp, C.c_char_p, ll]),
     "fdm_hubert_create": (ci, [ci, ci, ci, C.POINTER(vp)]),
diff --git a/face-diffusion-model_amd/fdm_amd/denoiser.py b/face-diffusion-model_amd/fdm_amd/denoiser.py
--- a/face-diffusion-model_amd/fdm_amd/denoiser.py
+++ b/face-diffusion-model_amd/fdm_amd/denoiser.py
@@ -6,6 +6,7 @@
 from ._lib import F32, FdmError, ModelDesc, SampleArgs, check, lib
 
 TILE_SITES = ("enc", "qkv", "qkv_ln", "out", "out_ln", "ffn1", "ffn2", "ffn2_stat", "dec", "dec_ln")
+SHAPE_SITES = ("attn", "ln12", "ln3")
 
 
 def _dev(t, device):
@@ -475,7 +476,7 @@
 
     @property
     def tiles(self):
-        return {k: self.get("tile." + k) for k in TILE_SITES}
+        return {k: self.get("tile." + k) for k in TILE_SITES + SHAPE_SITES}
 
     @property
     def fuse_ln3(self):
diff --git a/face-diffusion-model_amd/fdm_amd/ops.py b/face-diffusion-model_amd/fdm_amd/ops.py
--- a/face-diffusion-model_amd/fdm_amd/ops.py
+++ b/face-diffusion-model_amd/fdm_amd/ops.py
@@ -127,7 +127,7 @@
     check(lib().fdm_op_pack_kv(_p(K), ldk, _p(V), ldv, _p(Kp), _p(Vp), B, H, L, Lpad, hd, code_of(K), stream()))
 
 
-def attention(Q, Kp, Vp, O, *, B, H, L, hd, ldq, ldo, Lpad, scale, causal=False, slopes=None, period=1, lens=None):
+def attention(Q, Kp, Vp, O, *, B, H, L, hd, ldq, ldo, Lpad, scale, causal=False, slopes=None, period=1, lens=None, qs=0):
     a = AttnArgs()
     a.Q, a.ldq, a.Kp, a.Vp, a.Lpad = _p(Q), ldq, _p(Kp), _p(Vp), Lpad
     a.O, a.ldo, a.B, a.H, a.L, a.hd, a.dtype = _p(O), ldo, B, H, L, hd, code_of(Q)
@@ -136,12 +136,13 @@
     elif isinstance(O, Split):
         a.o_split, a.o_lo_off = O.code, O.lo_off
     a.scale, a.causal, a.slopes, a.period, a.lens = scale, int(causal), _p(slopes), period, _p(lens)
+    a.qs = qs
     check(lib().fdm_op_attention(C.byref(a), stream()))
 
 
 def layernorm(x, gamma, beta, M, d, *, add_mat=None, add_tab=None, tab_index=None, tab_step=None, eps=1e-5,
               act=ACT_NONE, y_f32=None, y_t=None, dtype=F32, gamma2=None, beta2=None, x_planes=0, x_plane_stride=0,
-              clip_step=None, clip_step_stride=1, clip_rows=0, clip_wrap=0, add_mat_group=0, add_mat_wrap=0, add_mat_L=0):
+              clip_step=None, clip_step_stride=1, clip_rows=0, clip_wrap=0, add_mat_group=0, add_mat_wrap=0, add_mat_L=0, shape=0):
     a = LnArgs()
     a.x, a.M, a.d, a.add_mat, a.add_tab = _p(x), M, d, _p(add_mat), _p(add_tab)
     a.tab_index, a.tab_step, a.gamma, a.beta, a.eps = _p(tab_index), _p(tab_step), _p(gamma), _p(beta), eps
@@ -149,6 +150,7 @@
     a.gamma2, a.beta2, a.y_t_lo_off = _p(gamma2), _p(beta2), _lo(y_t)
     a.x_planes, a.x_plane_stride = x_planes, x_plane_stride
     a.add_mat_group, a.add_mat_wrap, a.add_mat_L = add_mat_group, add_mat_wrap, add_mat_L
+    a.shape = shape
     if clip_step is not None:
         a.clip_step, a.clip_step_stride, a.clip_rows, a.clip_wrap = _p(clip_step), clip_step_stride, clip_rows, clip_wrap
     check(lib().fdm_op_layernorm(C.byref(a), stream()))
diff --git a/include/fdm_hip.h b/include/fdm_hip.h
--- a/include/fdm_hip.h
+++ b/include/fdm_hip.h
@@ -120,6 +120,7 @@
   const void* Q; long long ldq;
   const void* Kp;
   const void* Vp; int Lpad;
+  int qs;
   void* O; long long ldo;
   int B, H, L, hd;
   int dtype;
@@ -143,6 +144,7 @@
   const float* gamma; const float* beta; float eps;
   int act;
   float* y_f32; void* y_t; int dtype;
+  int shape;
   const float* gamma2; const float* beta2;
   long long y_t_lo_off;
   int add_mat_L, add_mat_group, add_mat_wrap;
@@ -281,6 +283,7 @@
                                int L_total, int overlap, const float* x_T, unsigned long long seed, int clip_id, int sampler,
                                float cfg_scale, void* stream);
 int fdm_plan_tune(fdm_plan* p, void* stream);
+int fdm_tile_set_text(const char* sites, char* out, int cap);
 int fdm_plan_get(fdm_plan* p, const char* key, long long* out);
 int fdm_plan_set(fdm_plan* p, const char* key, long long value);
 
```

New measurement: 1920 frames/s. 3.1% lower.
